# ShuhangGu/DASR

Hardware: NVIDIA B200
Metric: x4 SR output megapixels/sec (RRDBNet-23 G forward) (higher is better)
Workload: dtype bf16

## Files before the change

### dasr_b200/csrc/conv_tc.cu

```cuda
#include <stdlib.h>
#include "tc_common.cuh"

namespace dasr {

constexpr int EPI_WGS = 2;
constexpr int EPI_WARPS = 4 * EPI_WGS;
constexpr int MMA_WARPS = 1;
constexpr int TCK_WARPS = 2 + EPI_WARPS + 1 + (MMA_WARPS - 1);
constexpr int TCK_THREADS = 32 * TCK_WARPS;

struct EpiMaps {
  CUtensorMap m[8];
};

struct TcKernelArgs {
  DasrConvTcParams p;
  const float* bias;
  const __nv_bfloat16* res1;
  const __nv_bfloat16* res2;
  const __nv_bfloat16* mask_src;
  void* out;
  int nchunks;
  int chunk64;
  int nloads;
  int n_ntiles;
  int tiles_x, tiles_y;
  long ntiles;
  int stages;
  int w_bytes;
  int a_stage_bytes;
  int tmem_cols;
  int nacc;
  int acc_stride;
  int epi_bytes;
  int has_pre, has_res1, has_res2;
  int nbuf;
};


template <int EPI_MODE, bool HAS_PRE, int NRES>
__global__ void __launch_bounds__(TCK_THREADS, 1)
conv_tc_kernel(const __grid_constant__ CUtensorMap tmap_in, const __grid_constant__ CUtensorMap tmap_w,
               const __grid_constant__ EpiMaps em, const TcKernelArgs a) {
  extern __shared__ __align__(1024) uint8_t smem_raw[];
  uint8_t* smem = reinterpret_cast<uint8_t*>((reinterpret_cast<uintptr_t>(smem_raw) + 1023) & ~uintptr_t(1023));
  uint8_t* sW = smem;
  uint8_t* sA = smem + a.w_bytes;
  const int nbuf = a.nbuf;
  uint8_t* sS = sA + (size_t)a.stages * a.a_stage_bytes;
  uint8_t* sR1 = sS + nbuf * a.epi_bytes;
  uint8_t* sR2 = sR1 + (NRES >= 1 ? nbuf * a.epi_bytes : 0);
  uint64_t* bars = reinterpret_cast<uint64_t*>(sR2 + (NRES >= 2 ? nbuf * a.epi_bytes : 0));
  uint64_t* full_bar = bars;
  uint64_t* empty_bar = bars + MAX_STAGES;
  uint64_t* w_bar = bars + 2 * MAX_STAGES;
  uint64_t* tfull_bar = bars + 2 * MAX_STAGES + 1;
  uint64_t* tempty_bar = bars + 2 * MAX_STAGES + 5;
  uint64_t* pre_bar = bars + 2 * MAX_STAGES + 9;
  uint64_t* sfull_bar = bars + 2 * MAX_STAGES + 13;
  uint64_t* sfree_bar = bars + 2 * MAX_STAGES + 17;
  uint32_t* tmem_ptr = reinterpret_cast<uint32_t*>(bars + 2 * MAX_STAGES + 21);
  float* sBias = reinterpret_cast<float*>(bars + 2 * MAX_STAGES + 22);

  const DasrConvTcParams& p = a.p;
  const int warp = threadIdx.x >> 5, lane = threadIdx.x & 31;
  const int var = blockIdx.y / a.n_ntiles;
  const int ntile = blockIdx.y - var * a.n_ntiles;
  const int nt = p.nt;
  const int ntaps = p.ntaps;
  const int acc_stride = a.acc_stride;
  const uint32_t nacc = (uint32_t)a.nacc;
  const int nb64 = nt >> 6;
  const bool tail32 = (nt & 32) != 0;
  const bool has_loads = (EPI_MODE == 0) && (HAS_PRE || NRES > 0);

  if (threadIdx.x == 0) {
    tma_prefetch_desc(&tmap_in);
    tma_prefetch_desc(&tmap_w);
    for (int s = 0; s < a.stages; s++) {
      mbar_init(&full_bar[s], 1);
      mbar_init(&empty_bar[s], 1);
    }
    mbar_init(w_bar, 1);
    for (int b = 0; b < 4; b++) {
      mbar_init(&tfull_bar[b], 1);
      mbar_init(&tempty_bar[b], EPI_WARPS);
    }
    for (int b = 0; b < 4; b++) {
      mbar_init(&pre_bar[b], 1);
      mbar_init(&sfull_bar[b], EPI_WARPS);
      mbar_init(&sfree_bar[b], 1);
    }
    fence_barrier_init();
  }
  if (warp == 1) tmem_alloc(tmem_ptr, (uint32_t)a.tmem_cols);
  for (int i = threadIdx.x; i < nt; i += TCK_THREADS) sBias[i] = a.bias ? a.bias[ntile * nt + i] : 0.f;
  tc_fence_before();
  __syncthreads();
  tc_fence_after();
  const uint32_t tmem_base = *tmem_ptr;
  pdl_launch_dependents();

  if (warp == 0) {
    if (lane == 0) {
      mbar_expect_tx(w_bar, (uint32_t)a.w_bytes);
      for (int tap = 0; tap < ntaps; tap++)
        for (int c = 0; c < a.nchunks; c++) {
          int slot = tap * a.nchunks + c;
          int row = ((var * ntaps + tap) * a.nchunks + c) * p.cout + ntile * nt;
          tma_load_2d(sW + (size_t)slot * nt * ROW_B, &tmap_w, w_bar, 0, row);
        }
    }
    int stage = 0;
    uint32_t phase = 0;
    if (lane == 0) pdl_wait();
    __syncwarp();
    for (long tile = blockIdx.x; tile < a.ntiles; tile += gridDim.x) {
      const uint32_t te = (uint32_t)(p.tile_rev ? a.ntiles - 1 - tile : tile);
      const uint32_t r = te / (uint32_t)a.tiles_x;
      const int tx = (int)(te - r * (uint32_t)a.tiles_x);
      const int n = (int)(r / (uint32_t)a.tiles_y);
      const int ty = (int)(r - (uint32_t)n * (uint32_t)a.tiles_y);
      int x0 = tx * TILE_W, y0 = ty * TILE_H;
      if (lane == 0) {
        for (int c = 0; c < a.nloads; c++) {
          mbar_wait(&empty_bar[stage], phase ^ 1);
          uint8_t* dst = sA + (size_t)stage * a.a_stage_bytes;
          if (a.chunk64) {
            mbar_expect_tx(&full_bar[stage], 2 * A_HALO_BYTES);
            tma_load_4d(dst, &tmap_in, &full_bar[stage], p.in_coff + c * 2 * CHUNK, x0 - 1, y0 - 1, n);
          } else if (p.a_mode == 0) {
            mbar_expect_tx(&full_bar[stage], A_HALO_BYTES);
            tma_load_4d(dst, &tmap_in, &full_bar[stage], p.nchunk_list ? p.chunk_off[c] : p.in_coff + c * CHUNK, x0 - 1, y0 - 1, n);
          } else {
            mbar_expect_tx(&full_bar[stage], (uint32_t)(ntaps * A_TAP_BYTES));
            for (int tap = 0; tap < ntaps; tap++)
              tma_load_4d(dst + (size_t)tap * A_TAP_BYTES, &tmap_in, &full_bar[stage], p.nchunk_list ? p.chunk_off[c] : p.in_coff + c * CHUNK,
                          x0 - 1 + p.tap_dx[var][tap], y0 - 1 + p.tap_dy[var][tap], n);
          }
          if (++stage == a.stages) { stage = 0; phase ^= 1; }
        }
      }
      __syncwarp();
    }
  } else if (warp == 1 || (MMA_WARPS > 1 && warp == TCK_WARPS - 1)) {
    const uint32_t mi = (warp == 1) ? 0u : 1u;
    const uint32_t idesc = make_idesc_16(128, nt, p.f16);
    const uint32_t a_row = a.chunk64 ? 2u * ROW_B : (uint32_t)ROW_B;
    const uint32_t a_sbo = (p.a_mode == 0 && EPI_MODE != 3) ? (uint32_t)HALO_W * a_row : 8u * a_row;
    const uint64_t a_hi = ((uint64_t)((a_sbo >> 4) & 0x3FFF) << 32) | ((uint64_t)1 << 46) | ((uint64_t)(a.chunk64 ? 2 : 4) << 61) | ((uint64_t)1 << 16);
    const int ksteps = a.chunk64 ? 4 : 2;
    const uint64_t b_hi = ((uint64_t)(((8 * ROW_B) >> 4) & 0x3FFF) << 32) | ((uint64_t)1 << 46) | ((uint64_t)4 << 61) | ((uint64_t)1 << 16);
    const uint32_t a_lo0 = smem_u32(sA) >> 4;
    const uint32_t a_stage_lo = (uint32_t)a.a_stage_bytes >> 4;
    const uint32_t b_lo0 = smem_u32(sW) >> 4;
    const uint32_t b_slot_lo = (uint32_t)(nt * ROW_B) >> 4;
    uint32_t tap_lo[9];
#pragma unroll
    for (int t = 0; t < 9; t++) {
      int tt = t < ntaps ? t : 0;
      tap_lo[t] = (p.a_mode == 0) ? ((uint32_t)(p.tap_dy[var][tt] * HALO_W + p.tap_dx[var][tt]) * a_row) >> 4
                                  : (uint32_t)(tt * A_TAP_BYTES) >> 4;
    }
    mbar_wait(w_bar, 0);
    tc_fence_after();
    int stage = 0;
    uint32_t phase = 0;
    uint32_t it = 0;
    for (long tile = blockIdx.x; tile < a.ntiles; tile += gridDim.x, it++) {
      if ((it % MMA_WARPS) != mi) {
        for (int c = 0; c < a.nloads; c++)
          if (++stage == a.stages) { stage = 0; phase ^= 1; }
        continue;
      }
      const int acc = (int)(it % nacc);
      const uint32_t acc_phase = (it / nacc) & 1;
      mbar_wait(&tempty_bar[acc], acc_phase ^ 1);
      tc_fence_after();
      const uint32_t d_tmem = tmem_base + (uint32_t)(acc * acc_stride);
      for (int c = 0; c < a.nloads; c++) {
        mbar_wait(&full_bar[stage], phase);
        tc_fence_after();
        if (elect_one()) {
          const uint32_t a_lo = a_lo0 + (uint32_t)stage * a_stage_lo;
          const uint32_t b_tap_step = (uint32_t)a.nchunks * b_slot_lo;
          const uint32_t cb = a.chunk64 ? 2u * (uint32_t)c : (uint32_t)c;
          if constexpr (EPI_MODE == 3) {
#pragma unroll
            for (int mh = 0; mh < 2; mh++) {
              const uint32_t al = a_lo + (uint32_t)mh * ((128u * a_row) >> 4);
              for (int ks = 0; ks < ksteps; ks++) {
                const uint32_t bl = b_lo0 + (cb + (uint32_t)(ks >> 1)) * b_slot_lo + 2u * (uint32_t)(ks & 1);
                umma_bf16(d_tmem + (uint32_t)mh * 32u, a_hi | (uint64_t)((al + 2u * ks) & 0x3FFF), b_hi | (uint64_t)(bl & 0x3FFF), idesc,
                          (uint32_t)((c | ks) != 0));
              }
            }
          } else {
#pragma unroll
            for (int tap = 0; tap < 9; tap++) {
              if (tap < ntaps) {
                const uint32_t al = a_lo + tap_lo[tap];
                for (int ks = 0; ks < ksteps; ks++) {
                  const uint32_t bl = b_lo0 + (cb + (uint32_t)(ks >> 1)) * b_slot_lo + (uint32_t)tap * b_tap_step + 2u * (uint32_t)(ks & 1);
                  umma_bf16(d_tmem, a_hi | (uint64_t)((al + 2u * ks) & 0x3FFF), b_hi | (uint64_t)(bl & 0x3FFF), idesc,
                            (uint32_t)((c | tap | ks) != 0));
                }
              }
            }
          }
          umma_commit(&empty_bar[stage]);
          if (c == a.nloads - 1) umma_commit(&tfull_bar[acc]);
        }
        __syncwarp();
        if (++stage == a.stages) { stage = 0; phase ^= 1; }
      }
    }
  } else if (warp == TCK_WARPS - MMA_WARPS) {
    if constexpr (EPI_MODE == 0) {
      const int co_base = p.out_coff + ntile * nt;
      const int omap = (p.out_mul == 2) ? 2 * var : 0;
      const uint32_t load_bytes = (uint32_t)(((HAS_PRE ? 1 : 0) + NRES) * a.epi_bytes);
      pdl_wait();
      auto tile_xyz = [&](long tile, int& x0, int& y0, int& n) {
        const uint32_t te = (uint32_t)(p.tile_rev ? a.ntiles - 1 - tile : tile);
        const uint32_t r = te / (uint32_t)a.tiles_x;
        const int tx = (int)(te - r * (uint32_t)a.tiles_x);
        n = (int)(r / (uint32_t)a.tiles_y);
        const int ty = (int)(r - (uint32_t)n * (uint32_t)a.tiles_y);
        x0 = tx * TILE_W;
        y0 = ty * TILE_H;
      };
      auto issue_loads = [&](long tile, int b) {
        int x0, y0, n;
        tile_xyz(tile, x0, y0, n);
        if (lane == 0) {
          mbar_expect_tx(&pre_bar[b], load_bytes);
          const int cb = ntile * nt;
          for (int i = 0; i < nb64 + (tail32 ? 1 : 0); i++) {
            const int wide = i < nb64;
            const int off = wide ? i * EPI_BLK64_BYTES : nb64 * EPI_BLK64_BYTES;
            const int col = cb + (wide ? i * 64 : nb64 * 64);
            if constexpr (HAS_PRE) tma_load_4d(sS + b * a.epi_bytes + off, &em.m[wide ? 2 : 3], &pre_bar[b], p.pre_coff + col, x0, y0, n);
            if constexpr (NRES >= 1) tma_load_4d(sR1 + b * a.epi_bytes + off, &em.m[wide ? 4 : 5], &pre_bar[b], p.res1_coff + col, x0, y0, n);
            if constexpr (NRES >= 2) tma_load_4d(sR2 + b * a.epi_bytes + off, &em.m[wide ? 6 : 7], &pre_bar[b], p.res2_coff + col, x0, y0, n);
          }
        }
        __syncwarp();
      };
      const long G = gridDim.x;
      if (has_loads) {
        for (int k = 0; k < nbuf; k++)
          if ((long)blockIdx.x + k * G < a.ntiles) issue_loads(blockIdx.x + k * G, k);
      }
      uint32_t it = 0;
      long prev_tile = -1;
      int prev_b = 0;
      auto retire = [&](long t, int bb) {
        if (has_loads) {
          if (t + (long)nbuf * G < a.ntiles) issue_loads(t + (long)nbuf * G, bb);
        } else if (lane == 0) {
          mbar_arrive(&sfree_bar[bb]);
        }
        __syncwarp();
      };
      for (long tile = blockIdx.x; tile < a.ntiles; tile += G, it++) {
        const int b = (int)(it % (uint32_t)nbuf);
        if (lane == 0) {
          int x0, y0, n;
          tile_xyz(tile, x0, y0, n);
          mbar_wait(&sfull_bar[b], (it / (uint32_t)nbuf) & 1);
          for (int i = 0; i < nb64 + (tail32 ? 1 : 0); i++) {
            const int wide = i < nb64;
            const int off = wide ? i * EPI_BLK64_BYTES : nb64 * EPI_BLK64_BYTES;
            tma_store_4d(&em.m[(wide ? 0 : 1) + omap], sS + b * a.epi_bytes + off, co_base + (wide ? i * 64 : nb64 * 64), x0, y0, n);
          }
          bulk_commit();
          if (prev_tile >= 0) asm volatile("cp.async.bulk.wait_group.read 1;" ::: "memory");
        }
        __syncwarp();
        if (prev_tile >= 0) retire(prev_tile, prev_b);
        prev_tile = tile;
        prev_b = b;
      }
      if (prev_tile >= 0) {
        if (lane == 0) bulk_wait_read0();
        __syncwarp();
        retire(prev_tile, prev_b);
      }
      if (lane == 0) bulk_wait0();
    }
  } else {
    if constexpr (EPI_MODE != 0) pdl_wait();
    const int ew = warp - 2;
    const int wg = ew >> 2;
    const int q = warp & 3;
    const int m = q * 32 + lane;
    const int py = m >> 3, px = m & 7;
    const int co_base = ntile * nt;
    const int OW = p.W * p.out_mul, OH = p.H * p.out_mul;
    const int ngroups = nt >> 4;
    const int act = p.act, f16 = p.f16;
    const float slope = p.slope, alpha = p.alpha;
    const bool scale = alpha != 1.f;
    const int sw64 = (m >> 1) & 3, sw128 = m & 7;
    const uint32_t sS_u = smem_u32(sS), sR1_u = smem_u32(sR1), sR2_u = smem_u32(sR2), sBias_u = smem_u32(sBias);
    const bool has_bias = a.bias != nullptr;
    uint32_t it = 0;
    const int g0 = wg, gs = EPI_WGS;
    for (long tile = blockIdx.x; tile < a.ntiles; tile += gridDim.x, it++) {
      const int acc = (int)(it % nacc);
      const uint32_t acc_phase = (it / nacc) & 1;
      const uint32_t te = (uint32_t)(p.tile_rev ? a.ntiles - 1 - tile : tile);
      const uint32_t r = te / (uint32_t)a.tiles_x;
      const int tx = (int)(te - r * (uint32_t)a.tiles_x);
      const int n = (int)(r / (uint32_t)a.tiles_y);
      const int ty = (int)(r - (uint32_t)n * (uint32_t)a.tiles_y);
      const int y = ty * TILE_H + py, x = tx * TILE_W + px;
      const bool valid = (y < p.H) && (x < p.W);
      const int oy = y * p.out_mul + p.out_py[var], ox = x * p.out_mul + p.out_px[var];
      const long opix = ((long)n * OH + oy) * OW + ox;
      const int sb = (int)(it % (uint32_t)nbuf);
      const uint32_t sphase = (it / (uint32_t)nbuf) & 1;
      const uint32_t bS = sS_u + sb * a.epi_bytes, bR1 = sR1_u + sb * a.epi_bytes, bR2 = sR2_u + sb * a.epi_bytes;

      mbar_wait(&tfull_bar[acc], acc_phase);
      tc_fence_after();
      if constexpr (EPI_MODE == 0) {
        if (has_loads) mbar_wait(&pre_bar[sb], sphase);
        else if (it >= (uint32_t)nbuf) mbar_wait(&sfree_bar[sb], sphase ^ 1);
      }
      const uint32_t t_addr = tmem_base + ((uint32_t)(q * 32) << 16) + (uint32_t)(acc * acc_stride);
      if constexpr (EPI_MODE == 3) {
        float* S = reinterpret_cast<float*>(sS);
        constexpr int SROW = 29;
        const int hrow = wg * 128 + m;
        uint32_t r0[16], r1[16];
        tmem_ld16(t_addr + wg * 32, r0);
        tmem_ld16(t_addr + wg * 32 + 16, r1);
        tmem_ld_wait();
        tc_fence_before();
        __syncwarp();
        if (lane == 0) mbar_arrive(&tempty_bar[acc]);
        if (hrow < HALO_W * HALO_H) {
#pragma unroll
          for (int j = 0; j < 16; j++) S[hrow * SROW + j] = __uint_as_float(r0[j]);
#pragma unroll
          for (int j = 0; j < 11; j++) S[hrow * SROW + 16 + j] = __uint_as_float(r1[j]);
        }
        asm volatile("bar.sync 1, %0;" ::"n"(EPI_WARPS * 32) : "memory");
        if (wg == 0 && valid) {
          float* of = reinterpret_cast<float*>(a.out);
          const long plane = (long)OH * OW;
          const int onc = p.out_nc;
          for (int c = 0; c < onc; c++) {
            float v = has_bias ? sBias[c] : 0.f;
#pragma unroll
            for (int t9 = 0; t9 < 9; t9++) v += S[((py + t9 / 3) * HALO_W + (px + t9 % 3)) * SROW + t9 * onc + c];
            if (act != DASR_ACT_NONE && p.act_cols > 0) v = (act == DASR_ACT_LRELU) ? fmaxf(v, v * slope) : fmaxf(v, 0.f);
            of[((long)n * onc + c) * plane + (long)oy * OW + ox] = v * alpha;
          }
        }
        asm volatile("bar.sync 1, %0;" ::"n"(EPI_WARPS * 32) : "memory");
        continue;
      }
      auto process = [&](const uint32_t* rr, int g) {
        const int cg = g << 4;
        const int co = co_base + cg;
        const bool do_act = (act != DASR_ACT_NONE) && (co + 16 <= p.act_cols);
        float v[16];
#pragma unroll
        for (int j = 0; j < 16; j++) v[j] = __uint_as_float(rr[j]);
        if (has_bias) {
#pragma unroll
          for (int j4 = 0; j4 < 4; j4++) {
            const float4 b4 = lds128f(sBias_u + (cg + 4 * j4) * 4);
            v[4 * j4 + 0] += b4.x;
            v[4 * j4 + 1] += b4.y;
            v[4 * j4 + 2] += b4.z;
            v[4 * j4 + 3] += b4.w;
          }
        }
        if constexpr (EPI_MODE == 0) {
          int o0, o1;
          if (cg < (nb64 << 6)) {
            const int base = (cg >> 6) * EPI_BLK64_BYTES + m * 128;
            const int c0 = (cg & 63) >> 3;
            o0 = base + ((c0 ^ sw128) << 4);
            o1 = base + (((c0 + 1) ^ sw128) << 4);
          } else {
            const int base = nb64 * EPI_BLK64_BYTES + m * 64;
            const int c0 = (cg & 31) >> 3;
            o0 = base + ((c0 ^ sw64) << 4);
            o1 = base + (((c0 + 1) ^ sw64) << 4);
          }
          if constexpr (HAS_PRE) {
            fma_h16x8(v, lds128(bS + o0), 1.f, f16);
            fma_h16x8(v + 8, lds128(bS + o1), 1.f, f16);
          }
          if (do_act) {
            if (act == DASR_ACT_LRELU) {
#pragma unroll
              for (int j = 0; j < 16; j++) v[j] = fmaxf(v[j], v[j] * slope);
            } else {
#pragma unroll
              for (int j = 0; j < 16; j++) v[j] = fmaxf(v[j], 0.f);
            }
          }
          if (scale) {
#pragma unroll
            for (int j = 0; j < 16; j++) v[j] *= alpha;
          }
          if constexpr (NRES >= 1) {
            fma_h16x8(v, lds128(bR1 + o0), p.beta1, f16);
            fma_h16x8(v + 8, lds128(bR1 + o1), p.beta1, f16);
          }
          if constexpr (NRES >= 2) {
            fma_h16x8(v, lds128(bR2 + o0), p.beta2, f16);
            fma_h16x8(v + 8, lds128(bR2 + o1), p.beta2, f16);
          }
          uint4 o[2];
          pack_h16x16(v, o, f16);
          sts128(bS + o0, o[0]);
          sts128(bS + o1, o[1]);
        } else if (valid) {
          if (do_act) {
#pragma unroll
            for (int j = 0; j < 16; j++) v[j] = (act == DASR_ACT_LRELU) ? fmaxf(v[j], v[j] * slope) : fmaxf(v[j], 0.f);
          }
#pragma unroll
          for (int j = 0; j < 16; j++) v[j] *= alpha;
          if constexpr (EPI_MODE == 2) {
            float* of = reinterpret_cast<float*>(a.out);
            const long plane = (long)OH * OW;
#pragma unroll
            for (int j = 0; j < 16; j++)
              if (co + j < p.out_nc) of[((long)n * p.out_nc + co + j) * plane + (long)oy * OW + ox] = v[j];
          } else {
            __nv_bfloat16* ob16 = reinterpret_cast<__nv_bfloat16*>(a.out);
            if (a.res1) {
              const uint4* rp = reinterpret_cast<const uint4*>(a.res1 + opix * p.res1_cs + p.res1_coff + co);
              fma_h16x8(v, __ldg(rp), p.beta1, f16);
              fma_h16x8(v + 8, __ldg(rp + 1), p.beta1, f16);
            }
            if (a.res2) {
              const uint4* rp = reinterpret_cast<const uint4*>(a.res2 + opix * p.res2_cs + p.res2_coff + co);
              fma_h16x8(v, __ldg(rp), p.beta2, f16);
              fma_h16x8(v + 8, __ldg(rp + 1), p.beta2, f16);
            }
            if (a.mask_src && co + 16 > p.mask_c0 && co < p.mask_c1) {
              const __nv_bfloat16* mp = a.mask_src + opix * p.mask_cs + p.mask_coff + (co - p.mask_c0);
#pragma unroll
              for (int j = 0; j < 16; j++) {
                int cc = co + j;
                if (cc >= p.mask_c0 && cc < p.mask_c1) {
                  float mv = __bfloat162float(mp[j]);
                  if (!(mv > 0.f)) v[j] *= p.mask_slope;
                }
              }
            }
            uint4 o[2];
            pack_h16x16(v, o, f16);
            uint4* op = reinterpret_cast<uint4*>(ob16 + opix * p.out_cs + p.out_coff + co);
            op[0] = o[0];
            op[1] = o[1];
          }
        }
      };
      auto release_acc = [&]() {
        tc_fence_before();
        __syncwarp();
        if (lane == 0) mbar_arrive(&tempty_bar[acc]);
      };
      uint32_t ra[16], rb[16];
      if (g0 < ngroups) tmem_ld16(t_addr + g0 * 16, ra);
      for (int g = g0; g < ngroups; g += 2 * gs) {
        tmem_ld_wait();
        if (g + gs < ngroups) tmem_ld16(t_addr + (g + gs) * 16, rb); else release_acc();
        process(ra, g);
        if (g + gs < ngroups) {
          tmem_ld_wait();
          if (g + 2 * gs < ngroups) tmem_ld16(t_addr + (g + 2 * gs) * 16, ra); else release_acc();
          process(rb, g + gs);
        }
      }
      if (g0 >= ngroups) {
        tc_fence_before();
        __syncwarp();
        if (lane == 0) mbar_arrive(&tempty_bar[acc]);
      }
      if constexpr (EPI_MODE == 0) {
        fence_proxy_async();
        __syncwarp();
        if (lane == 0) mbar_arrive(&sfull_bar[sb]);
      }
    }
  }

  tc_fence_before();
  __syncthreads();
  if (warp == 1) {
    tc_fence_after();
    tmem_dealloc(tmem_base, (uint32_t)a.tmem_cols);
  }
}

__global__ void pack_filter_tc_kernel(const float* __restrict__ w, unsigned short* __restrict__ o, int cout, int cin,
                                      int kind, int f16) {
  const int gn = (kind == 1) ? cin : cout;
  const int gk = (kind == 1) ? cout : cin;
  if (kind == 3) {
    const long total3 = (long)(cin / CHUNK) * 32 * CHUNK;
    const long i3 = (long)blockIdx.x * blockDim.x + threadIdx.x;
    if (i3 >= total3) return;
    const int kc3 = (int)(i3 % CHUNK), n3 = (int)((i3 / CHUNK) % 32), c3 = (int)(i3 / (CHUNK * 32));
    float v3 = 0.f;
    if (n3 < 9 * cout) {
      const int tap = n3 / cout, co = n3 - tap * cout;
      v3 = w[((long)co * cin + c3 * CHUNK + kc3) * 9 + tap];
    }
    o[i3] = f16 ? __half_as_ushort(__float2half_rn(v3)) : __bfloat16_as_ushort(__float2bfloat16(v3));
    return;
  }
  const int nvar = (kind == 2) ? 4 : 1, ntaps = (kind == 2) ? 4 : 9, nchunks = gk / CHUNK;
  long total = (long)nvar * ntaps * nchunks * gn * CHUNK;
  long i = (long)blockIdx.x * blockDim.x + threadIdx.x;
  if (i >= total) return;
  int kc = (int)(i % CHUNK);
  long r = i / CHUNK;
  int nn = (int)(r % gn); r /= gn;
  int c = (int)(r % nchunks); r /= nchunks;
  int tap = (int)(r % ntaps);
  int var = (int)(r / ntaps);
  int kk = c * CHUNK + kc;
  float v = 0.f;
  if (kind == 0) {
    v = w[((long)nn * cin + kk) * 9 + tap];
  } else if (kind == 1) {
    int dy = tap / 3, dx = tap % 3;
    v = w[((long)kk * cin + nn) * 9 + (2 - dy) * 3 + (2 - dx)];
  } else {
    int py = var >> 1, px = var & 1, ta = tap >> 1, tb = tap & 1;
    int r0, r1, c0, c1;
    if (py == 0) { r0 = ta ? 1 : 0; r1 = ta ? 2 : 0; } else { r0 = ta ? 2 : 0; r1 = ta ? 2 : 1; }
    if (px == 0) { c0 = tb ? 1 : 0; c1 = tb ? 2 : 0; } else { c0 = tb ? 2 : 0; c1 = tb ? 2 : 1; }
    for (int rr = r0; rr <= r1; rr++)
      for (int cc = c0; cc <= c1; cc++) v += w[((long)nn * cin + kk) * 9 + rr * 3 + cc];
  }
  o[i] = f16 ? __half_as_ushort(__float2half_rn(v)) : __bfloat16_as_ushort(__float2bfloat16(v));
}

__global__ void pack_filter_tc_batch_kernel(const DasrPackJob* __restrict__ jobs) {
  const DasrPackJob j = jobs[blockIdx.y];
  if (j.kind == 3) {
    float* d = reinterpret_cast<float*>(j.dst);
    for (long i = (long)blockIdx.x * blockDim.x + threadIdx.x; i < j.cout; i += (long)gridDim.x * blockDim.x) d[i] = j.src[i];
    return;
  }
  const int rows = (j.kind == 1) ? j.ci_n : j.cout_rows;
  const int gk = (j.kind == 1) ? j.k_pad : j.ci_n;
  const int nvar = (j.kind == 2) ? 4 : 1, ntaps = (j.kind == 2) ? 4 : 9, nchunks = gk / CHUNK;
  const long total = (long)nvar * ntaps * nchunks * rows * CHUNK;
  __nv_bfloat16* o = reinterpret_cast<__nv_bfloat16*>(j.dst);
  for (long i = (long)blockIdx.x * blockDim.x + threadIdx.x; i < total; i += (long)gridDim.x * blockDim.x) {
    int kc = (int)(i % CHUNK);
    long r = i / CHUNK;
    int nn = (int)(r % rows); r /= rows;
    int c = (int)(r % nchunks); r /= nchunks;
    int tap = (int)(r % ntaps);
    int var = (int)(r / ntaps);
    int kk = c * CHUNK + kc;
    float v = 0.f;
    if (j.kind == 0) {
      if (nn < j.cout && j.ci_lo + kk < j.cin) v = j.src[((long)nn * j.cin + j.ci_lo + kk) * 9 + tap];
    } else if (j.kind == 1) {
      int dy = tap / 3, dx = tap % 3;
      if (kk < j.cout && j.ci_lo + nn < j.cin) v = j.src[((long)kk * j.cin + j.ci_lo + nn) * 9 + (2 - dy) * 3 + (2 - dx)];
    } else {
      int py = var >> 1, px = var & 1, ta = tap >> 1, tb = tap & 1;
      int r0, r1, c0, c1;
      if (py == 0) { r0 = ta ? 1 : 0; r1 = ta ? 2 : 0; } else { r0 = ta ? 2 : 0; r1 = ta ? 2 : 1; }
      if (px == 0) { c0 = tb ? 1 : 0; c1 = tb ? 2 : 0; } else { c0 = tb ? 2 : 0; c1 = tb ? 2 : 1; }
      if (nn < j.cout && j.ci_lo + kk < j.cin)
        for (int rr = r0; rr <= r1; rr++)
          for (int cc = c0; cc <= c1; cc++) v += j.src[((long)nn * j.cin + j.ci_lo + kk) * 9 + rr * 3 + cc];
    }
    o[(((long)var * ntaps + tap) * nchunks + c) * j.dst_rows * CHUNK + (long)(j.dst_row_off + nn) * CHUNK + kc] = __float2bfloat16(v);
  }
}


static int pow2_at_least(int v) {
  int r = 32;
  while (r < v) r <<= 1;
  return r;
}


__global__ void __launch_bounds__(128, 1) mma_rate_kernel(int n, int sbo, int iters, int a_step, long long* out) {
  const int nacc = (a_step >> 16) & 15 ? (a_step >> 16) & 15 : 1;
  const bool nowait = (a_step >> 20) & 1;
  a_step &= 0xFFFF;
  extern __shared__ __align__(1024) uint8_t smem_raw[];
  uint8_t* smem = reinterpret_cast<uint8_t*>((reinterpret_cast<uintptr_t>(smem_raw) + 1023) & ~uintptr_t(1023));
  __shared__ uint64_t bar;
  __shared__ uint32_t tptr;
  for (int i = threadIdx.x; i < 48 * 1024 / 4; i += blockDim.x) reinterpret_cast<uint32_t*>(smem)[i] = 0;
  if (threadIdx.x == 0) { mbar_init(&bar, 1); fence_barrier_init(); }
  fence_proxy_async();
  if (threadIdx.x < 32) tmem_alloc(&tptr, 512);
  tc_fence_before();
  __syncthreads();
  tc_fence_after();
  const uint32_t tb = tptr;
  if (threadIdx.x < 32) {
    const uint32_t idesc = make_idesc_bf16(128, n);
    const uint32_t a0 = smem_u32(smem), b0 = smem_u32(smem + 16384);
    const uint32_t acc_stride = 512u / (uint32_t)nacc;
    long long t0 = clock64();
    uint32_t ph = 0;
    for (int it = 0; it < iters; it++) {
      if (elect_one()) {
        int kk = 0;
#pragma unroll 1
        for (int tap = 0; tap < 9; tap++) {
          uint32_t aa = a0 + (uint32_t)(((tap / 3) * 10 + (tap % 3)) * a_step);
#pragma unroll
          for (int k = 0; k < 2; k++, kk++)
            umma_bf16(tb + (uint32_t)(kk % nacc) * acc_stride, make_desc_sw64(aa + k * 32, (uint32_t)sbo),
                      make_desc_sw64(b0 + k * 32, 512), idesc, 1u);
        }
        if (!nowait || it == iters - 1) umma_commit(&bar);
      }
      __syncwarp();
      if (!nowait || it == iters - 1) {
        mbar_wait(&bar, ph);
        ph ^= 1;
      }
    }
    long long t1 = clock64();
    if (threadIdx.x == 0 && blockIdx.x == 0) out[0] = (t1 - t0);
  }
  tc_fence_before();
  __syncthreads();
  if (threadIdx.x < 32) { tc_fence_after(); tmem_dealloc(tb, 512); }
}

__global__ void __launch_bounds__(64, 1) tma_rate_kernel(const __grid_constant__ CUtensorMap tm, int rows_per_box,
                                                         int box_bytes, int iters, int store, long npix, long long* out) {
  extern __shared__ __align__(1024) uint8_t smem_raw[];
  uint8_t* smem = reinterpret_cast<uint8_t*>((reinterpret_cast<uintptr_t>(smem_raw) + 1023) & ~uintptr_t(1023));
  __shared__ uint64_t bar[4];
  if (threadIdx.x == 0) {
    for (int i = 0; i < 4; i++) mbar_init(&bar[i], 1);
    fence_barrier_init();
  }
  __syncthreads();
  if (threadIdx.x == 0) {
    const int nbox = (int)(npix / rows_per_box);
    long long t0 = clock64();
    if (!store) {
      uint32_t ph[4] = {0, 0, 0, 0};
      for (int i = 0; i < iters + 4; i++) {
        int s = i & 3;
        if (i >= 4) { mbar_wait(&bar[s], ph[s]); ph[s] ^= 1; }
        if (i < iters) {
          int b = (int)(((long)blockIdx.x * 7919 + (long)i * 104729) % nbox);
          mbar_expect_tx(&bar[s], (uint32_t)box_bytes);
          tma_load_2d(smem + s * 49152, &tm, &bar[s], 0, b * rows_per_box);
        }
      }
    } else {
      for (int i = 0; i < iters; i++) {
        int b = (int)(((long)blockIdx.x * 7919 + (long)i * 104729) % nbox);
        asm volatile("cp.async.bulk.tensor.2d.global.shared::cta.bulk_group [%0, {%2, %3}], [%1];" ::"l"(
                         reinterpret_cast<uint64_t>(&tm)), "r"(smem_u32(smem + (i & 3) * 49152)), "r"(0), "r"(b * rows_per_box)
                     : "memory");
        bulk_commit();
        asm volatile("cp.async.bulk.wait_group.read 3;" ::: "memory");
      }
      bulk_wait0();
    }
    long long t1 = clock64();
    if (blockIdx.x == 0) out[0] = t1 - t0;
  }
}

}

using namespace dasr;

extern "C" {

int dasr_conv_tc_setup(DasrConvTcParams* p, int kind) {
  if (!p) return DASR_E_BADARG;
  p->nchunk_list = 0;
  p->f16 = 0;
  if (kind == 0 || kind == 1) {
    p->nvar = 1;
    p->ntaps = 9;
    p->out_mul = 1;
    for (int t = 0; t < 9; t++) {
      p->tap_dy[0][t] = (int8_t)(t / 3);
      p->tap_dx[0][t] = (int8_t)(t % 3);
    }
    p->out_py[0] = p->out_px[0] = 0;
  } else if (kind == 2) {
    p->nvar = 4;
    p->ntaps = 4;
    p->out_mul = 2;
    for (int v = 0; v < 4; v++) {
      int py = v >> 1, px = v & 1;
      p->out_py[v] = py;
      p->out_px[v] = px;
      for (int t = 0; t < 4; t++) {
        p->tap_dy[v][t] = (int8_t)(py + (t >> 1));
        p->tap_dx[v][t] = (int8_t)(px + (t & 1));
      }
    }
  } else if (kind == 3) {
    p->nvar = 1;
    p->ntaps = 1;
    p->out_mul = 1;
    p->tap_dy[0][0] = p->tap_dx[0][0] = 0;
    p->out_py[0] = p->out_px[0] = 0;
  } else {
    set_error("conv_tc_setup: unknown kind %d", kind);
    return DASR_E_BADARG;
  }
  return DASR_OK;
}

size_t dasr_pack_filter_tc_bytes(int cout, int cin, int kind) {
  if (kind == 3) return (size_t)(cin / CHUNK) * 32 * CHUNK * 2;
  int nvar = (kind == 2) ? 4 : 1, ntaps = (kind == 2) ? 4 : 9;
  return (size_t)nvar * ntaps * cout * cin * 2;
}

int dasr_pack_filter_tc(const float* w, void* o, int cout, int cin, int kind, void* stream) {
  const int f16 = (kind & DASR_TC_PACK_F16) != 0;
  kind &= ~DASR_TC_PACK_F16;
  DASR_REQUIRE(kind >= 0 && kind <= 3, "pack_filter_tc: kind");
  DASR_REQUIRE(kind != 3 || (cout >= 1 && 9 * cout <= 32), "pack_filter_tc: kind 3 (taps in N) needs cout <= 3");
  int gk = (kind == 1) ? cout : cin;
  DASR_REQUIRE(gk % CHUNK == 0, "pack_filter_tc: contraction channels (%d) must be a multiple of 32", gk);
  long total = (long)dasr_pack_filter_tc_bytes(cout, cin, kind) / 2;
  pack_filter_tc_kernel<<<cdiv(total, 256), 256, 0, (cudaStream_t)stream>>>(w, (unsigned short*)o, cout, cin, kind, f16);
  return check_launch("pack_filter_tc");
}

int dasr_pack_filter_tc_batch(const DasrPackJob* jobs_dev, int njobs, int blocks_per_job, void* stream) {
  DASR_REQUIRE(jobs_dev && njobs > 0 && njobs <= 65535 && blocks_per_job > 0, "pack_filter_tc_batch: bad arguments");
  dim3 grid(blocks_per_job, njobs);
  pack_filter_tc_batch_kernel<<<grid, 256, 0, (cudaStream_t)stream>>>(jobs_dev);
  return check_launch("pack_filter_tc_batch");
}

static int encode_act_map(PFN_encodeTiled enc, CUtensorMap* tm, const void* base, int cs, int W, int H, int N,
                          int width, const char* what, int mul = 1) {
  cuuint64_t gdim[4] = {(cuuint64_t)cs, (cuuint64_t)W, (cuuint64_t)H, (cuuint64_t)N};
  cuuint64_t gstr[3] = {(cuuint64_t)mul * cs * 2, (cuuint64_t)mul * (mul * W) * cs * 2, (cuuint64_t)(mul * H) * (mul * W) * cs * 2};
  cuuint32_t box[4] = {(cuuint32_t)width, TILE_W, TILE_H, 1};
  cuuint32_t estr[4] = {1, 1, 1, 1};
  CUresult r = enc(tm, CU_TENSOR_MAP_DATA_TYPE_BFLOAT16, 4, const_cast<void*>(base), gdim, gstr, box, estr,
                   CU_TENSOR_MAP_INTERLEAVE_NONE, width == 64 ? CU_TENSOR_MAP_SWIZZLE_128B : CU_TENSOR_MAP_SWIZZLE_64B,
                   (width == 32 && cs > 32) ? CU_TENSOR_MAP_L2_PROMOTION_L2_64B : CU_TENSOR_MAP_L2_PROMOTION_L2_128B,
                   CU_TENSOR_MAP_FLOAT_OOB_FILL_NONE);
  if (r != CUDA_SUCCESS) {
    set_error("conv_tc: cuTensorMapEncodeTiled(%s) failed: %d", what, (int)r);
    return DASR_E_LAUNCH;
  }
  return DASR_OK;
}

int dasr_conv_tc(const void* in, const void* w, const float* bias, const void* pre, const void* res1, const void* res2,
                 const void* mask_src, void* out, const DasrConvTcParams* p, void* stream) {
  DASR_REQUIRE(p && in && w && out, "conv_tc: null argument");
  DASR_REQUIRE(p->N > 0 && p->H > 0 && p->W > 0, "conv_tc: bad dims");
  DASR_REQUIRE((long)p->N * cdiv(p->W, TILE_W) * cdiv(p->H, TILE_H) < (1L << 30), "conv_tc: too many tiles for 32-bit tile arithmetic");
  DASR_REQUIRE(p->cin > 0 && p->cin % CHUNK == 0, "conv_tc: cin must be a multiple of 32 (got %d)", p->cin);
  if (p->nchunk_list > 0) {
    DASR_REQUIRE(p->nchunk_list <= 8 && p->nchunk_list * CHUNK == p->cin && p->in_cs % 8 == 0, "conv_tc: chunk list must cover cin");
    for (int i = 0; i < p->nchunk_list; i++)
      DASR_REQUIRE(p->chunk_off[i] >= 0 && p->chunk_off[i] % 8 == 0 && p->chunk_off[i] + CHUNK <= p->in_cs, "conv_tc: chunk_off[%d]", i);
  } else {
    DASR_REQUIRE(p->in_cs % 8 == 0 && p->in_coff % 8 == 0 && p->in_coff + p->cin <= p->in_cs, "conv_tc: input slice");
  }
  DASR_REQUIRE(p->nt >= 16 && p->nt <= 256 && p->nt % 16 == 0 && p->cout % p->nt == 0, "conv_tc: nt=%d cout=%d",
               p->nt, p->cout);
  DASR_REQUIRE(p->nvar >= 1 && p->nvar <= 4 && p->ntaps >= 1 && p->ntaps <= 9, "conv_tc: variants/taps");
  DASR_REQUIRE(p->out_mul == 1 || p->out_mul == 2, "conv_tc: out_mul");
  DASR_REQUIRE(p->epi_mode >= 0 && p->epi_mode <= 3, "conv_tc: epi_mode");
  DASR_REQUIRE(p->f16 == 0 || (p->f16 == 1 && !mask_src), "conv_tc: f16 must be 0/1; the dgrad mask input is bf16 only");
  DASR_REQUIRE(p->act_cols % 16 == 0, "conv_tc: act_cols must be a multiple of 16");
  if (p->epi_mode == 2) {
    DASR_REQUIRE(p->out_nc >= 1 && p->out_nc <= 16 && p->nt == p->cout && !res1 && !res2 && !pre && !mask_src,
                 "conv_tc: NCHW-fp32 epilogue supports out_nc<=16, one Cout tile, no residuals");
  } else if (p->epi_mode == 3) {
    DASR_REQUIRE(p->out_nc >= 1 && 9 * p->out_nc <= 32 && p->nt == 32 && p->cout == 32 && p->ntaps == 1 && p->nvar == 1 &&
                     p->a_mode == 0 && p->out_mul == 1 && !res1 && !res2 && !pre && !mask_src && !p->tile_rev,
                 "conv_tc: epi_mode 3 (taps in N, NCHW fp32 out) needs dasr_conv_tc_setup kind 3, out_nc <= 3, nt = cout = 32");
  } else {
    DASR_REQUIRE(p->out_cs % 8 == 0 && p->out_coff % 8 == 0 && p->out_coff + p->cout <= p->out_cs, "conv_tc: output slice");
  }
  if (p->epi_mode == 0) {
    DASR_REQUIRE(p->nt % 32 == 0 && !mask_src, "conv_tc: staged epilogue needs nt%%32==0, no mask");
    DASR_REQUIRE(p->out_mul == 1 || (!pre && !res1 && !res2),
                 "conv_tc: the staged epilogue of the sub-pixel (out_mul=2) variants has no pre / residual inputs");
  } else {
    DASR_REQUIRE(!pre, "conv_tc: the pre-activation addend is only supported by the staged epilogue (epi_mode 0)");
  }
  if (res1) DASR_REQUIRE(p->res1_cs % 8 == 0 && p->res1_coff % 8 == 0, "conv_tc: res1 alignment");
  if (res2) DASR_REQUIRE(p->res2_cs % 8 == 0 && p->res2_coff % 8 == 0, "conv_tc: res2 alignment");
  if (pre) DASR_REQUIRE(p->pre_cs % 8 == 0 && p->pre_coff % 8 == 0, "conv_tc: pre alignment");
  DASR_REQUIRE((reinterpret_cast<uintptr_t>(in) & 15) == 0 && (reinterpret_cast<uintptr_t>(out) & 15) == 0 &&
                   (reinterpret_cast<uintptr_t>(w) & 15) == 0,
               "conv_tc: pointers must be 16-byte aligned");
  PFN_encodeTiled enc = get_encode();
  if (!enc) {
    set_error("conv_tc: cuTensorMapEncodeTiled not available");
    return DASR_E_NODRIVER;
  }

  TcKernelArgs a;
  a.p = *p;
  a.bias = bias;
  a.res1 = (const __nv_bfloat16*)res1;
  a.res2 = (const __nv_bfloat16*)res2;
  a.mask_src = (const __nv_bfloat16*)mask_src;
  a.out = out;
  a.nchunks = p->cin / CHUNK;
  a.n_ntiles = p->cout / p->nt;
  a.tiles_x = cdiv(p->W, TILE_W);
  a.tiles_y = cdiv(p->H, TILE_H);
  a.ntiles = (long)p->N * a.tiles_x * a.tiles_y;
  a.w_bytes = p->ntaps * a.nchunks * p->nt * ROW_B;
  static int chunk64_ok = -1;
  if (chunk64_ok < 0) {
    const char* e = getenv("DASR_TC_CHUNK64");
    chunk64_ok = (e && e[0] == '0') ? 0 : 1;
  }
  a.chunk64 = (chunk64_ok && p->a_mode == 0 && p->nchunk_list == 0 && p->cin % (2 * CHUNK) == 0) ? 1 : 0;
  a.nloads = a.chunk64 ? a.nchunks / 2 : a.nchunks;
  a.a_stage_bytes = (p->a_mode == 0) ? (((a.chunk64 ? 2 : 1) * A_HALO_BYTES + 1023) / 1024 * 1024) : p->ntaps * A_TAP_BYTES;
  a.acc_stride = (p->epi_mode == 3) ? 64 : pow2_at_least(p->nt);
  a.nacc = (a.acc_stride <= 128) ? 4 : 2;
  a.tmem_cols = a.nacc * a.acc_stride;
  if (a.tmem_cols < 32) a.tmem_cols = 32;
  a.has_pre = (p->epi_mode == 0 && pre) ? 1 : 0;
  a.has_res1 = (p->epi_mode == 0 && res1) ? 1 : 0;
  a.has_res2 = (p->epi_mode == 0 && res2) ? 1 : 0;
  a.epi_bytes = (p->epi_mode == 0) ? p->nt * 128 * 2 : (p->epi_mode == 3 ? 21504 : 0);
  const int bar_bytes = (2 * MAX_STAGES + 22) * 8 + 256 * 4 + 16;
  int nbuf = (p->epi_mode == 0) ? 4 : (p->epi_mode == 3 ? 1 : 2);
  int epi_total = 0, avail = 0;
  for (;; nbuf--) {
    epi_total = nbuf * a.epi_bytes * (1 + a.has_res1 + a.has_res2);
    avail = SMEM_LIMIT - 1024  - a.w_bytes - epi_total - bar_bytes;
    if (nbuf <= 2 || avail >= 4 * a.a_stage_bytes) break;
  }
  a.nbuf = nbuf;
  int stages = avail / a.a_stage_bytes;
  if (stages > MAX_STAGES) stages = MAX_STAGES;
  if (stages < 2) {
    set_error("conv_tc: resident filters (%d B) + epilogue tiles (%d B) + 2 A stages do not fit shared memory; use a smaller nt",
              a.w_bytes, epi_total);
    return DASR_E_SMEM;
  }
  a.stages = stages;
  size_t smem = 1024 + (size_t)a.w_bytes + (size_t)stages * a.a_stage_bytes + epi_total + bar_bytes;
  if (smem < 120 * 1024) smem = 120 * 1024;

  CUtensorMap tm_in, tm_w;
  EpiMaps em;
  {
    cuuint64_t gdim[4] = {(cuuint64_t)p->in_cs, (cuuint64_t)p->W, (cuuint64_t)p->H, (cuuint64_t)p->N};
    cuuint64_t gstr[3] = {(cuuint64_t)p->in_cs * 2, (cuuint64_t)p->W * p->in_cs * 2,
                          (cuuint64_t)p->H * p->W * p->in_cs * 2};
    cuuint32_t box[4] = {(cuuint32_t)(a.chunk64 ? 2 * CHUNK : CHUNK), (cuuint32_t)(p->a_mode == 0 ? HALO_W : TILE_W),
                         (cuuint32_t)(p->a_mode == 0 ? HALO_H : TILE_H), 1};
    cuuint32_t estr[4] = {1, 1, 1, 1};
    CUresult r = enc(&tm_in, CU_TENSOR_MAP_DATA_TYPE_BFLOAT16, 4, const_cast<void*>(in), gdim, gstr, box, estr,
                     CU_TENSOR_MAP_INTERLEAVE_NONE, a.chunk64 ? CU_TENSOR_MAP_SWIZZLE_128B : CU_TENSOR_MAP_SWIZZLE_64B,
                     (p->in_cs > CHUNK && !a.chunk64) ? CU_TENSOR_MAP_L2_PROMOTION_L2_64B : CU_TENSOR_MAP_L2_PROMOTION_L2_128B,
                     CU_TENSOR_MAP_FLOAT_OOB_FILL_NONE);
    if (r != CUDA_SUCCESS) {
      set_error("conv_tc: cuTensorMapEncodeTiled(input) failed: %d", (int)r);
      return DASR_E_LAUNCH;
    }
  }
  {
    cuuint64_t rows = (cuuint64_t)p->nvar * p->ntaps * a.nchunks * p->cout;
    cuuint64_t gdim[2] = {CHUNK, rows};
    cuuint64_t gstr[1] = {ROW_B};
    cuuint32_t box[2] = {CHUNK, (cuuint32_t)p->nt};
    cuuint32_t estr[2] = {1, 1};
    CUresult r = enc(&tm_w, CU_TENSOR_MAP_DATA_TYPE_BFLOAT16, 2, const_cast<void*>(w), gdim, gstr, box, estr,
                     CU_TENSOR_MAP_INTERLEAVE_NONE, CU_TENSOR_MAP_SWIZZLE_64B, CU_TENSOR_MAP_L2_PROMOTION_L2_128B,
                     CU_TENSOR_MAP_FLOAT_OOB_FILL_NONE);
    if (r != CUDA_SUCCESS) {
      set_error("conv_tc: cuTensorMapEncodeTiled(filter) failed: %d", (int)r);
      return DASR_E_LAUNCH;
    }
  }
  for (int i = 0; i < 8; i++) em.m[i] = tm_in;
  if (p->epi_mode == 0) {
    const void* bases[4] = {out, pre, res1, res2};
    const int css[4] = {p->out_cs, p->pre_cs, p->res1_cs, p->res2_cs};
    const int used[4] = {1, a.has_pre, a.has_res1, a.has_res2};
    const char* names[4] = {"output", "pre", "res1", "res2"};
    if (p->out_mul == 2) {
      for (int v = 0; v < p->nvar && v < 4; v++) {
        const char* vb = (const char*)out + ((size_t)p->out_py[v] * (2 * p->W) + p->out_px[v]) * p->out_cs * 2;
        int rc;
        if (p->nt >= 64 && (rc = encode_act_map(enc, &em.m[2 * v], vb, p->out_cs, p->W, p->H, p->N, 64, "output", 2))) return rc;
        if ((p->nt & 32) && (rc = encode_act_map(enc, &em.m[2 * v + 1], vb, p->out_cs, p->W, p->H, p->N, 32, "output", 2))) return rc;
      }
    } else
    for (int t = 0; t < 4; t++) {
      if (!used[t]) continue;
      int rc;
      if (p->nt >= 64 && (rc = encode_act_map(enc, &em.m[2 * t], bases[t], css[t], p->W, p->H, p->N, 64, names[t]))) return rc;
      if ((p->nt & 32) && (rc = encode_act_map(enc, &em.m[2 * t + 1], bases[t], css[t], p->W, p->H, p->N, 32, names[t]))) return rc;
    }
  }

  typedef void (*KernelFn)(const CUtensorMap, const CUtensorMap, const EpiMaps, const TcKernelArgs);
  static const KernelFn kernels[9] = {
      conv_tc_kernel<0, false, 0>, conv_tc_kernel<0, false, 1>, conv_tc_kernel<0, false, 2>,
      conv_tc_kernel<0, true, 0>,  conv_tc_kernel<0, true, 1>,  conv_tc_kernel<0, true, 2>,
      conv_tc_kernel<1, false, 0>, conv_tc_kernel<2, false, 0>, conv_tc_kernel<3, false, 0>};
  const int ki = (p->epi_mode == 0) ? (a.has_pre * 3 + a.has_res1 + a.has_res2) : (5 + p->epi_mode);
  if (p->epi_mode == 0) DASR_REQUIRE(!(a.has_res2 && !a.has_res1), "conv_tc: res2 without res1");
  static bool attr_set[9] = {false, false, false, false, false, false, false, false, false};
  if (!attr_set[ki]) {
    cudaError_t e = cudaFuncSetAttribute(kernels[ki], cudaFuncAttributeMaxDynamicSharedMemorySize, SMEM_LIMIT);
    if (e != cudaSuccess) {
      set_error("conv_tc: cudaFuncSetAttribute: %s", cudaGetErrorString(e));
      return DASR_E_LAUNCH;
    }
    attr_set[ki] = true;
  }
  int gy = p->nvar * a.n_ntiles;
  int gx = num_sms() / gy;
  if (gx < 1) gx = 1;
  if ((long)gx > a.ntiles) gx = (int)a.ntiles;
  cudaLaunchConfig_t cfg = {};
  cfg.gridDim = dim3(gx, gy, 1);
  cfg.blockDim = dim3(TCK_THREADS, 1, 1);
  cfg.dynamicSmemBytes = smem;
  cfg.stream = (cudaStream_t)stream;
  cudaLaunchAttribute attrs[1];
  attrs[0].id = cudaLaunchAttributeProgrammaticStreamSerialization;
  attrs[0].val.programmaticStreamSerializationAllowed = pdl_enabled() ? 1 : 0;
  cfg.attrs = attrs;
  cfg.numAttrs = 1;
  cudaError_t le = cudaLaunchKernelEx(&cfg, kernels[ki], tm_in, tm_w, em, a);
  if (le != cudaSuccess) {
    set_error("conv_tc: launch failed: %s", cudaGetErrorString(le));
    return DASR_E_LAUNCH;
  }
  return check_launch("conv_tc");
}

int dasr_probe_mma_rate(int n, int sbo, int iters, int a_step, double* cycles_per_mma) {
  long long* d;
  if (cudaMalloc(&d, 8) != cudaSuccess) return DASR_E_LAUNCH;
  cudaFuncSetAttribute(mma_rate_kernel, cudaFuncAttributeMaxDynamicSharedMemorySize, 64 * 1024);
  mma_rate_kernel<<<num_sms(), 128, 64 * 1024>>>(n, sbo, iters, a_step, d);
  long long h = 0;
  cudaError_t e = cudaMemcpy(&h, d, 8, cudaMemcpyDeviceToHost);
  cudaFree(d);
  if (e != cudaSuccess) { set_error("probe: %s", cudaGetErrorString(e)); return DASR_E_LAUNCH; }
  *cycles_per_mma = (double)h / ((double)iters * 18.0);
  return DASR_OK;
}


int dasr_probe_tma_rate(int row_elems, int rows_per_box, int cs, int store, double* cycles_per_box) {
  PFN_encodeTiled enc = get_encode();
  if (!enc) return DASR_E_NODRIVER;
  const long npix = 1L << 20;
  void* buf;
  if (cudaMalloc(&buf, (size_t)npix * cs * 2) != cudaSuccess) return DASR_E_LAUNCH;
  cudaMemset(buf, 0, (size_t)npix * cs * 2);
  CUtensorMap tm;
  cuuint64_t gdim[2] = {(cuuint64_t)cs, (cuuint64_t)npix};
  cuuint64_t gstr[1] = {(cuuint64_t)cs * 2};
  cuuint32_t box[2] = {(cuuint32_t)row_elems, (cuuint32_t)rows_per_box};
  cuuint32_t estr[2] = {1, 1};
  CUtensorMapSwizzle sw = row_elems * 2 == 64 ? CU_TENSOR_MAP_SWIZZLE_64B : (row_elems * 2 == 128 ? CU_TENSOR_MAP_SWIZZLE_128B : CU_TENSOR_MAP_SWIZZLE_NONE);
  CUresult r = enc(&tm, CU_TENSOR_MAP_DATA_TYPE_BFLOAT16, 2, buf, gdim, gstr, box, estr, CU_TENSOR_MAP_INTERLEAVE_NONE, sw,
                   CU_TENSOR_MAP_L2_PROMOTION_L2_128B, CU_TENSOR_MAP_FLOAT_OOB_FILL_NONE);
  if (r != CUDA_SUCCESS) { cudaFree(buf); set_error("probe tma: encode %d", (int)r); return DASR_E_LAUNCH; }
  long long* d;
  cudaMalloc(&d, 8);
  const int iters = 400;
  cudaFuncSetAttribute(tma_rate_kernel, cudaFuncAttributeMaxDynamicSharedMemorySize, 200 * 1024);
  tma_rate_kernel<<<num_sms(), 64, 200 * 1024>>>(tm, rows_per_box, row_elems * 2 * rows_per_box, iters, store, npix, d);
  long long h = 0;
  cudaError_t e = cudaMemcpy(&h, d, 8, cudaMemcpyDeviceToHost);
  cudaFree(d);
  cudaFree(buf);
  if (e != cudaSuccess) { set_error("probe tma: %s", cudaGetErrorString(e)); return DASR_E_LAUNCH; }
  *cycles_per_box = (double)h / iters;
  return DASR_OK;
}

}
```

### dasr_b200/csrc/conv_tc2.cu

```cuda
#include <stdlib.h>
#include "tc_common.cuh"

namespace dasr {

constexpr int TC2_EPI_WARPS = 8;
constexpr int TC2_WARPS = 2 + TC2_EPI_WARPS + 1;
constexpr int TC2_THREADS = 32 * TC2_WARPS;
constexpr int TC2_MAX_STAGES = 6;
constexpr int TC2_MAX_BLOCKS = 6;

struct Tc2Maps {
  CUtensorMap m[8];
};

struct Tc2Args {
  DasrConvTcParams p;
  const float* bias;
  int nchunks;
  int n_half;
  int tiles_x, tiles_y;
  long ntiles;
  int stages, a_stage_bytes, w_bytes;
  int nblk;
  int nb64;
  int nb;
  int acc_stride;
};

template <bool HAS_PRE, int NRES>
__global__ void __cluster_dims__(2, 1, 1) __launch_bounds__(TC2_THREADS, 1)
conv_tc2_kernel(const __grid_constant__ CUtensorMap tmap_in, const __grid_constant__ CUtensorMap tmap_w,
                const __grid_constant__ Tc2Maps em, const Tc2Args a) {
  extern __shared__ __align__(1024) uint8_t smem_raw[];
  uint8_t* smem = reinterpret_cast<uint8_t*>((reinterpret_cast<uintptr_t>(smem_raw) + 1023) & ~uintptr_t(1023));
  uint8_t* sW = smem;
  uint8_t* sA = smem + a.w_bytes;
  uint8_t* sS = sA + (size_t)a.stages * a.a_stage_bytes;
  uint8_t* sR1 = sS + (size_t)a.nblk * EPI_BLK64_BYTES;
  uint8_t* sR2 = sR1 + (NRES >= 1 ? (size_t)a.nblk * EPI_BLK64_BYTES : 0);
  uint64_t* bars = reinterpret_cast<uint64_t*>(sR2 + (NRES >= 2 ? (size_t)a.nblk * EPI_BLK64_BYTES : 0));
  constexpr bool HAS_LOADS = HAS_PRE || NRES > 0;
  uint64_t* full_bar = bars;
  uint64_t* empty_bar = bars + TC2_MAX_STAGES;
  uint64_t* w_bar = bars + 2 * TC2_MAX_STAGES;
  uint64_t* tfull_bar = w_bar + 1;
  uint64_t* tempty_bar = tfull_bar + 2;
  uint64_t* sfull_bar = tempty_bar + 2;
  uint64_t* sfree_bar = sfull_bar + TC2_MAX_BLOCKS;
  uint64_t* pre_bar = sfree_bar + TC2_MAX_BLOCKS;
  uint32_t* tmem_ptr = reinterpret_cast<uint32_t*>(pre_bar + TC2_MAX_BLOCKS);
  float* sBias = reinterpret_cast<float*>(bars + 40);

  const DasrConvTcParams& p = a.p;
  const int warp = threadIdx.x >> 5, lane = threadIdx.x & 31;
  const uint32_t rank = cluster_ctarank();
  const long pair = blockIdx.x >> 1, npairs = gridDim.x >> 1;
  const int cout = p.nt;
  const int co_base = (int)blockIdx.y * p.nt;

  if (threadIdx.x == 0) {
    tma_prefetch_desc(&tmap_in);
    tma_prefetch_desc(&tmap_w);
    tma_prefetch_desc(&em.m[0]);
    for (int s = 0; s < a.stages; s++) {
      mbar_init(&full_bar[s], 1);
      mbar_init(&empty_bar[s], 1);
    }
    mbar_init(w_bar, 1);
    for (int b = 0; b < 2; b++) {
      mbar_init(&tfull_bar[b], 1);
      mbar_init(&tempty_bar[b], 2 * TC2_EPI_WARPS);
    }
    for (int b = 0; b < a.nblk; b++) {
      mbar_init(&sfull_bar[b], TC2_EPI_WARPS);
      mbar_init(&sfree_bar[b], 1);
      mbar_init(&pre_bar[b], 1);
    }
    fence_barrier_init();
  }
  for (int i = threadIdx.x; i < cout; i += TC2_THREADS) sBias[i] = a.bias ? a.bias[co_base + i] : 0.f;
  cluster_sync();
  if (warp == 1) tmem_alloc2(tmem_ptr, 512);
  tc_fence_before();
  __syncthreads();
  tc_fence_after();
  const uint32_t tmem_base = *tmem_ptr;
  pdl_launch_dependents();

  auto tile_of = [&](long it, int& x0, int& y0, int& n) -> bool {
    uint32_t t = 2u * (uint32_t)(pair + it * npairs) + rank;
    const bool live = (long)t < a.ntiles;
    if (p.tile_rev && live) t = (uint32_t)(a.ntiles - 1) - t;
    const uint32_t r = t / (uint32_t)a.tiles_x;
    const uint32_t tx = t - r * (uint32_t)a.tiles_x;
    n = (int)(r / (uint32_t)a.tiles_y);
    const uint32_t ty = r - (uint32_t)n * (uint32_t)a.tiles_y;
    x0 = (int)tx * TILE_W;
    y0 = (int)ty * TILE_H;
    return live;
  };
  const long niter = (a.ntiles / 2 + (a.ntiles & 1) - pair + npairs - 1) / npairs;

  if (warp == 0) {
    if (lane == 0) {
      if (rank == 0) mbar_expect_tx(w_bar, 2u * (uint32_t)a.w_bytes);
      for (int tap = 0; tap < 9; tap++)
        for (int c = 0; c < a.nchunks; c++) {
          const int slot = tap * a.nchunks + c;
          const int row = slot * p.cout + co_base + (int)rank * a.n_half;
          tma2_load_2d(sW + (size_t)slot * a.n_half * ROW_B, &tmap_w, w_bar, 0, row);
        }
      pdl_wait();
      int stage = 0;
      uint32_t phase = 0;
      for (long it = 0; it < niter; it++) {
        int x0, y0, n;
        tile_of(it, x0, y0, n);
        for (int c = 0; c < a.nchunks; c++) {
          mbar_wait(&empty_bar[stage], phase ^ 1);
          if (rank == 0) mbar_expect_tx(&full_bar[stage], 2u * A_HALO_BYTES);
          tma2_load_4d(sA + (size_t)stage * a.a_stage_bytes, &tmap_in, &full_bar[stage],
                       p.nchunk_list ? p.chunk_off[c] : p.in_coff + c * CHUNK, x0 - 1, y0 - 1, n);
          if (++stage == a.stages) { stage = 0; phase ^= 1; }
        }
      }
    }
    __syncwarp();
  } else if (warp == 1) {
    if (rank == 0) {
      const uint32_t idesc = make_idesc_16(256, cout, p.f16);
      const uint32_t a_sbo = (uint32_t)(HALO_W * ROW_B);
      const uint64_t a_hi = ((uint64_t)((a_sbo >> 4) & 0x3FFF) << 32) | ((uint64_t)1 << 46) | ((uint64_t)4 << 61) | ((uint64_t)1 << 16);
      const uint64_t b_hi = ((uint64_t)(((8 * ROW_B) >> 4) & 0x3FFF) << 32) | ((uint64_t)1 << 46) | ((uint64_t)4 << 61) | ((uint64_t)1 << 16);
      const uint32_t a_lo0 = smem_u32(sA) >> 4;
      const uint32_t a_stage_lo = (uint32_t)a.a_stage_bytes >> 4;
      const uint32_t b_lo0 = smem_u32(sW) >> 4;
      const uint32_t b_slot_lo = (uint32_t)(a.n_half * ROW_B) >> 4;
      uint32_t tap_lo[9];
#pragma unroll
      for (int t = 0; t < 9; t++) tap_lo[t] = (uint32_t)(((t / 3) * HALO_W + (t % 3)) * ROW_B) >> 4;
      mbar_wait(w_bar, 0);
      tc_fence_after();
      int stage = 0;
      uint32_t phase = 0;
      for (long it = 0; it < niter; it++) {
        const int acc = (int)(it & 1);
        mbar_wait(&tempty_bar[acc], ((uint32_t)(it >> 1) & 1) ^ 1);
        tc_fence_after();
        const uint32_t d_tmem = tmem_base + (uint32_t)(acc * a.acc_stride);
        for (int c = 0; c < a.nchunks; c++) {
          mbar_wait(&full_bar[stage], phase);
          tc_fence_after();
          if (elect_one()) {
            const uint32_t a_lo = a_lo0 + (uint32_t)stage * a_stage_lo;
            uint32_t b_lo = b_lo0 + (uint32_t)c * b_slot_lo;
            const uint32_t b_tap_step = (uint32_t)a.nchunks * b_slot_lo;
#pragma unroll
            for (int tap = 0; tap < 9; tap++) {
              const uint32_t al = a_lo + tap_lo[tap];
              umma2_bf16(d_tmem, a_hi | (uint64_t)(al & 0x3FFF), b_hi | (uint64_t)(b_lo & 0x3FFF), idesc, (uint32_t)((c | tap) != 0));
              umma2_bf16(d_tmem, a_hi | (uint64_t)((al + 2) & 0x3FFF), b_hi | (uint64_t)((b_lo + 2) & 0x3FFF), idesc, 1u);
              b_lo += b_tap_step;
            }
            umma2_commit_mc(&empty_bar[stage]);
            if (c == a.nchunks - 1) umma2_commit_mc(&tfull_bar[acc]);
          }
          __syncwarp();
          if (++stage == a.stages) { stage = 0; phase ^= 1; }
        }
      }
    }
  } else if (warp == TC2_WARPS - 1) {
    if (lane == 0) {
      pdl_wait();
      const uint32_t nb = (uint32_t)a.nb, nblk = (uint32_t)a.nblk;
      const uint32_t total = (uint32_t)niter * nb;
      const uint32_t nld = (uint32_t)((HAS_PRE ? 1 : 0) + NRES);
      const bool mask_mode = (NRES >= 1) && (p.mask_c1 > p.mask_c0);
      auto issue_loads = [&](uint32_t k) {
        const uint32_t b = k % nblk;
        int x0, y0, n;
        const uint32_t kt = k / nb;
        tile_of((long)kt, x0, y0, n);
        const int i = (int)(k - kt * nb);
        const int wide = i < a.nb64 ? 1 : 0;
        const int col = co_base + i * 64;
        const bool need_r1 = !mask_mode || (col < p.mask_c1 && col + (wide ? 64 : 32) > p.mask_c0);
        mbar_expect_tx(&pre_bar[b], (nld - (need_r1 ? 0u : 1u)) * (uint32_t)(wide ? EPI_BLK64_BYTES : EPI_BLK32_BYTES));
        if constexpr (HAS_PRE) tma_load_4d(sS + (size_t)b * EPI_BLK64_BYTES, &em.m[wide ? 2 : 3], &pre_bar[b], p.pre_coff + col, x0, y0, n);
        if constexpr (NRES >= 1) {
          if (need_r1) tma_load_4d(sR1 + (size_t)b * EPI_BLK64_BYTES, &em.m[wide ? 4 : 5], &pre_bar[b], p.res1_coff + col, x0, y0, n);
        }
        if constexpr (NRES >= 2) tma_load_4d(sR2 + (size_t)b * EPI_BLK64_BYTES, &em.m[wide ? 6 : 7], &pre_bar[b], p.res2_coff + col, x0, y0, n);
      };
      if constexpr (HAS_LOADS)
        for (uint32_t k = 0; k < nblk && k < total; k++) issue_loads(k);
      auto retire = [&](uint32_t k) {
        if constexpr (HAS_LOADS) {
          if (k + nblk < total) issue_loads(k + nblk);
        } else {
          mbar_arrive(&sfree_bar[k % nblk]);
        }
      };
      int x0 = 0, y0 = 0, n = 0;
      bool live = false;
      uint32_t i = 0;
      for (uint32_t k = 0; k < total; k++) {
        const uint32_t b = k % nblk;
        if (i == 0) live = tile_of((long)(k / nb), x0, y0, n);
        mbar_wait(&sfull_bar[b], (k / nblk) & 1);
        if (live) tma_store_4d(&em.m[(int)i < a.nb64 ? 0 : 1], sS + (size_t)b * EPI_BLK64_BYTES, p.out_coff + co_base + (int)i * 64, x0, y0, n);
        bulk_commit();
        if (k >= 1) {
          asm volatile("cp.async.bulk.wait_group.read 1;" ::: "memory");
          retire(k - 1);
        }
        if (++i == nb) i = 0;
      }
      if (total > 0) {
        bulk_wait_read0();
        retire(total - 1);
      }
      bulk_wait0();
    }
    __syncwarp();
  } else {
    const int ew = warp - 2;
    const int wg = ew >> 2;
    const int q = warp & 3;
    const int m = q * 32 + lane;
    const int sw128 = m & 7, sw64 = (m >> 1) & 3;
    const int act = p.act, f16 = p.f16;
    const float slope = p.slope, alpha = p.alpha;
    const bool scale = alpha != 1.f;
    const uint32_t sS_u = smem_u32(sS), sR1_u = smem_u32(sR1), sR2_u = smem_u32(sR2), sBias_u = smem_u32(sBias);
    const bool has_bias = a.bias != nullptr;
    uint32_t k = 0;
    for (long it = 0; it < niter; it++) {
      const int acc = (int)(it & 1);
      mbar_wait(&tfull_bar[acc], (uint32_t)(it >> 1) & 1);
      tc_fence_after();
      const uint32_t t_addr = tmem_base + ((uint32_t)(q * 32) << 16) + (uint32_t)(acc * a.acc_stride);
      for (int i = 0; i < a.nb; i++, k++) {
        const int b = (int)(k % (uint32_t)a.nblk);
        if constexpr (HAS_LOADS) {
          mbar_wait(&pre_bar[b], (k / (uint32_t)a.nblk) & 1);
        } else {
          if (k >= (uint32_t)a.nblk) mbar_wait(&sfree_bar[b], ((k / (uint32_t)a.nblk) & 1) ^ 1);
        }
        const bool wide = i < a.nb64;
        const uint32_t rowoff = (uint32_t)m * (wide ? 128u : 64u);
        const uint32_t bS = sS_u + (uint32_t)b * EPI_BLK64_BYTES + rowoff;
        const uint32_t bR1 = sR1_u + (uint32_t)b * EPI_BLK64_BYTES + rowoff;
        const uint32_t bR2 = sR2_u + (uint32_t)b * EPI_BLK64_BYTES + rowoff;
        uint32_t ra[16], rb[16];
        const int c0 = i * 64 + wg * 16, c1 = c0 + 32;
        tmem_ld16(t_addr + c0, ra);
        if (wide) tmem_ld16(t_addr + c1, rb);
        tmem_ld_wait();
        if (i == a.nb - 1) {
          tc_fence_before();
          __syncwarp();
          if (lane == 0) mbar_arrive_leader(&tempty_bar[acc]);
        }
#pragma unroll
        for (int h = 0; h < 2; h++) {
          if (h == 1 && !wide) break;
          const uint32_t* rr = h ? rb : ra;
          const int cg = h ? c1 : c0;
          const bool do_act = (act != DASR_ACT_NONE) && (co_base + cg + 16 <= p.act_cols);
          float v[16];
#pragma unroll
          for (int j = 0; j < 16; j++) v[j] = __uint_as_float(rr[j]);
          if (has_bias) {
#pragma unroll
            for (int j4 = 0; j4 < 4; j4++) {
              const float4 b4 = lds128f(sBias_u + (cg + 4 * j4) * 4);
              v[4 * j4 + 0] += b4.x;
              v[4 * j4 + 1] += b4.y;
              v[4 * j4 + 2] += b4.z;
              v[4 * j4 + 3] += b4.w;
            }
          }
          const int ch = (cg & (wide ? 63 : 31)) >> 3;
          const int sw = wide ? sw128 : sw64;
          const uint32_t o0 = (uint32_t)(((ch) ^ sw) << 4), o1 = (uint32_t)(((ch + 1) ^ sw) << 4);
          if constexpr (HAS_PRE) {
            fma_h16x8(v, lds128(bS + o0), 1.f, f16);
            fma_h16x8(v + 8, lds128(bS + o1), 1.f, f16);
          }
          if (do_act) {
            if (act == DASR_ACT_LRELU) {
#pragma unroll
              for (int j = 0; j < 16; j++) v[j] = fmaxf(v[j], v[j] * slope);
            } else {
#pragma unroll
              for (int j = 0; j < 16; j++) v[j] = fmaxf(v[j], 0.f);
            }
          }
          if (scale) {
#pragma unroll
            for (int j = 0; j < 16; j++) v[j] *= alpha;
          }
          if constexpr (NRES >= 1) {
            if (p.mask_c1 > p.mask_c0) {
              const int co = co_base + cg;
              if (co >= p.mask_c0 && co < p.mask_c1) {
                const uint4 m0 = lds128(bR1 + o0), m1 = lds128(bR1 + o1);
                const short* ms0 = reinterpret_cast<const short*>(&m0);
                const short* ms1 = reinterpret_cast<const short*>(&m1);
#pragma unroll
                for (int j = 0; j < 8; j++) {
                  if (!(ms0[j] > 0)) v[j] *= p.mask_slope;
                  if (!(ms1[j] > 0)) v[8 + j] *= p.mask_slope;
                }
              }
            } else {
              fma_h16x8(v, lds128(bR1 + o0), p.beta1, f16);
              fma_h16x8(v + 8, lds128(bR1 + o1), p.beta1, f16);
            }
          }
          if constexpr (NRES >= 2) {
            fma_h16x8(v, lds128(bR2 + o0), p.beta2, f16);
            fma_h16x8(v + 8, lds128(bR2 + o1), p.beta2, f16);
          }
          uint4 o[2];
          pack_h16x16(v, o, f16);
          sts128(bS + o0, o[0]);
          sts128(bS + o1, o[1]);
        }
        fence_proxy_async();
        __syncwarp();
        if (lane == 0) mbar_arrive(&sfull_bar[b]);
      }
    }
  }

  tc_fence_before();
  cluster_sync();
  if (warp == 1) {
    tc_fence_after();
    tmem_dealloc2(tmem_base, 512);
  }
}

__global__ void __cluster_dims__(2, 1, 1) __launch_bounds__(128, 1) mma2_rate_kernel(int n, int iters, long long* out) {
  extern __shared__ __align__(1024) uint8_t smem_raw[];
  uint8_t* smem = reinterpret_cast<uint8_t*>((reinterpret_cast<uintptr_t>(smem_raw) + 1023) & ~uintptr_t(1023));
  __shared__ uint64_t bar;
  __shared__ uint32_t tptr;
  for (int i = threadIdx.x; i < 48 * 1024 / 4; i += blockDim.x) reinterpret_cast<uint32_t*>(smem)[i] = 0;
  if (threadIdx.x == 0) { mbar_init(&bar, 1); fence_barrier_init(); }
  fence_proxy_async();
  cluster_sync();
  if (threadIdx.x < 32) tmem_alloc2(&tptr, 512);
  tc_fence_before();
  __syncthreads();
  tc_fence_after();
  const uint32_t tb = tptr;
  const uint32_t rank = cluster_ctarank();
  if (threadIdx.x < 32 && rank == 0) {
    const uint32_t idesc = make_idesc_bf16(256, n);
    const uint32_t a0 = smem_u32(smem), b0 = smem_u32(smem + 16384);
    long long t0 = clock64();
    for (int it = 0; it < iters; it++) {
      if (elect_one()) {
#pragma unroll 1
        for (int tap = 0; tap < 9; tap++) {
          uint32_t aa = a0 + (uint32_t)(((tap / 3) * 10 + (tap % 3)) * 64);
#pragma unroll
          for (int k = 0; k < 2; k++)
            umma2_bf16(tb, make_desc_sw64(aa + k * 32, 640), make_desc_sw64(b0 + k * 32, 512), idesc, 1u);
        }
        if (it == iters - 1)
          asm volatile("tcgen05.commit.cta_group::2.mbarrier::arrive::one.shared::cluster.b64 [%0];" ::"r"(smem_u32(&bar)) : "memory");
      }
      __syncwarp();
    }
    mbar_wait(&bar, 0);
    long long t1 = clock64();
    if (threadIdx.x == 0 && blockIdx.x == 0) out[0] = (t1 - t0);
  }
  tc_fence_before();
  cluster_sync();
  if (threadIdx.x < 32) { tc_fence_after(); tmem_dealloc2(tb, 512); }
}

}

using namespace dasr;

extern "C" {

static int tc2_plan(const DasrConvTcParams* p, int has_pre, int nres, int* stages_out, int* nblk_out) {
  const int nchunks = p->cin / CHUNK;
  const long w_bytes = (long)9 * nchunks * (p->nt / 2) * ROW_B;
  const int a_stage = (A_HALO_BYTES + 1023) / 1024 * 1024;
  const int bar_bytes = 40 * 8 + 256 * 4 + 64;
  const int per_blk = (1 + nres) * EPI_BLK64_BYTES;
  (void)has_pre;
  static int force_nblk = -1;
  if (force_nblk < 0) {
    const char* e = getenv("DASR_TC2_NBLK");
    force_nblk = e ? atoi(e) : 0;
  }
  for (int want = 4; want >= 2; want--)
    for (int nblk = TC2_MAX_BLOCKS; nblk >= 2; nblk--) {
      if (force_nblk > 0 && nblk != force_nblk) continue;
      const long avail = (long)SMEM_LIMIT - 1024 - w_bytes - (long)nblk * per_blk - bar_bytes;
      int stages = (int)(avail / a_stage);
      if (stages > TC2_MAX_STAGES) stages = TC2_MAX_STAGES;
      if (stages >= want) {
        *stages_out = stages;
        *nblk_out = nblk;
        return 1;
      }
    }
  return 0;
}

int dasr_conv_tc2_supported(const DasrConvTcParams* p) {
  if (!p) return 0;
  if (p->nvar != 1 || p->ntaps != 9 || p->out_mul != 1 || p->epi_mode != 0 || p->a_mode != 0) return 0;
  if (p->nt % 32 != 0 || p->nt < 32 || p->nt > 256 || p->cout % p->nt != 0 || p->cin % CHUNK != 0 || p->cin <= 0) return 0;
  int st, nb;
  const int nres = (p->res1_cs > 0 ? 1 : 0) + (p->res2_cs > 0 ? 1 : 0);
  return tc2_plan(p, p->pre_cs > 0 ? 1 : 0, nres, &st, &nb);
}

int dasr_conv_tc2(const void* in, const void* w, const float* bias, const void* pre, const void* res1, const void* res2,
                  void* out, const DasrConvTcParams* p, void* stream) {
  DASR_REQUIRE(p && in && w && out, "conv_tc2: null argument");
  DASR_REQUIRE(p->nvar == 1 && p->ntaps == 9 && p->out_mul == 1 && p->epi_mode == 0 && p->a_mode == 0,
               "conv_tc2: plain 3x3 geometry with the staged epilogue only");
  DASR_REQUIRE(p->nt % 32 == 0 && p->nt >= 32 && p->nt <= 256 && p->cout % p->nt == 0,
               "conv_tc2: the Cout tile nt must be a multiple of 32 in [32, 256] that divides cout (nt=%d cout=%d)", p->nt, p->cout);
  DASR_REQUIRE(p->N > 0 && p->H > 0 && p->W > 0, "conv_tc2: bad dims");
  DASR_REQUIRE((long)p->N * cdiv(p->W, TILE_W) * cdiv(p->H, TILE_H) < (1L << 30), "conv_tc2: too many tiles for 32-bit tile arithmetic");
  DASR_REQUIRE(p->cin > 0 && p->cin % CHUNK == 0, "conv_tc2: cin must be a multiple of 32 (got %d)", p->cin);
  if (p->nchunk_list > 0) {
    DASR_REQUIRE(p->nchunk_list <= 8 && p->nchunk_list * CHUNK == p->cin, "conv_tc2: chunk list must cover cin");
    for (int i = 0; i < p->nchunk_list; i++)
      DASR_REQUIRE(p->chunk_off[i] >= 0 && p->chunk_off[i] % 8 == 0 && p->chunk_off[i] + CHUNK <= p->in_cs, "conv_tc2: chunk_off[%d]", i);
  } else {
    DASR_REQUIRE(p->in_cs % 8 == 0 && p->in_coff % 8 == 0 && p->in_coff + p->cin <= p->in_cs, "conv_tc2: input slice");
  }
  DASR_REQUIRE(p->out_cs % 8 == 0 && p->out_coff % 8 == 0 && p->out_coff + p->cout <= p->out_cs, "conv_tc2: output slice");
  DASR_REQUIRE(p->act_cols % 16 == 0, "conv_tc2: act_cols must be a multiple of 16");
  DASR_REQUIRE(!(res2 && !res1), "conv_tc2: res2 without res1");
  if (p->mask_c1 > p->mask_c0)
    DASR_REQUIRE(res1 && !res2 && p->mask_c0 % 16 == 0 && p->mask_c1 % 16 == 0 && p->mask_c1 <= p->cout,
                 "conv_tc2: mask mode takes the activation as res1 (no res2) and a range of whole 16-channel groups");
  if (pre) DASR_REQUIRE(p->pre_cs % 8 == 0 && p->pre_coff % 8 == 0 && p->pre_coff + p->cout <= p->pre_cs, "conv_tc2: pre slice");
  if (res1) DASR_REQUIRE(p->res1_cs % 8 == 0 && p->res1_coff % 8 == 0 && p->res1_coff + p->cout <= p->res1_cs, "conv_tc2: res1 slice");
  if (res2) DASR_REQUIRE(p->res2_cs % 8 == 0 && p->res2_coff % 8 == 0 && p->res2_coff + p->cout <= p->res2_cs, "conv_tc2: res2 slice");
  PFN_encodeTiled enc = get_encode();
  if (!enc) {
    set_error("conv_tc2: cuTensorMapEncodeTiled not available");
    return DASR_E_NODRIVER;
  }
  const int has_pre = pre ? 1 : 0, nres = (res1 ? 1 : 0) + (res2 ? 1 : 0);
  Tc2Args a;
  a.p = *p;
  a.bias = bias;
  a.nchunks = p->cin / CHUNK;
  a.n_half = p->nt / 2;
  a.tiles_x = cdiv(p->W, TILE_W);
  a.tiles_y = cdiv(p->H, TILE_H);
  a.ntiles = (long)p->N * a.tiles_x * a.tiles_y;
  a.w_bytes = 9 * a.nchunks * a.n_half * ROW_B;
  a.a_stage_bytes = (A_HALO_BYTES + 1023) / 1024 * 1024;
  a.nb64 = p->nt / 64;
  a.nb = a.nb64 + ((p->nt & 32) ? 1 : 0);
  a.acc_stride = 256;
  const int bar_bytes = 40 * 8 + 256 * 4 + 64;
  int stages = 0, nblk = 0;
  if (!tc2_plan(p, has_pre, nres, &stages, &nblk)) {
    set_error("conv_tc2: filters (%d B per CTA) + %d epilogue block arrays do not fit shared memory", a.w_bytes, 1 + nres);
    return DASR_E_SMEM;
  }
  a.stages = stages;
  a.nblk = nblk;
  size_t smem = 1024 + (size_t)a.w_bytes + (size_t)stages * a.a_stage_bytes + (size_t)nblk * (1 + nres) * EPI_BLK64_BYTES + bar_bytes;
  if (smem < 120 * 1024) smem = 120 * 1024;

  CUtensorMap tm_in, tm_w;
  Tc2Maps em;
  {
    cuuint64_t gdim[4] = {(cuuint64_t)p->in_cs, (cuuint64_t)p->W, (cuuint64_t)p->H, (cuuint64_t)p->N};
    cuuint64_t gstr[3] = {(cuuint64_t)p->in_cs * 2, (cuuint64_t)p->W * p->in_cs * 2, (cuuint64_t)p->H * p->W * p->in_cs * 2};
    cuuint32_t box[4] = {CHUNK, HALO_W, HALO_H, 1};
    cuuint32_t estr[4] = {1, 1, 1, 1};
    CUresult r = enc(&tm_in, CU_TENSOR_MAP_DATA_TYPE_BFLOAT16, 4, const_cast<void*>(in), gdim, gstr, box, estr,
                     CU_TENSOR_MAP_INTERLEAVE_NONE, CU_TENSOR_MAP_SWIZZLE_64B,
                     p->in_cs > CHUNK ? CU_TENSOR_MAP_L2_PROMOTION_L2_64B : CU_TENSOR_MAP_L2_PROMOTION_L2_128B,
                     CU_TENSOR_MAP_FLOAT_OOB_FILL_NONE);
    if (r != CUDA_SUCCESS) { set_error("conv_tc2: cuTensorMapEncodeTiled(input) failed: %d", (int)r); return DASR_E_LAUNCH; }
  }
  {
    cuuint64_t rows = (cuuint64_t)9 * a.nchunks * p->cout;
    cuuint64_t gdim[2] = {CHUNK, rows};
    cuuint64_t gstr[1] = {ROW_B};
    cuuint32_t box[2] = {CHUNK, (cuuint32_t)a.n_half};
    cuuint32_t estr[2] = {1, 1};
    CUresult r = enc(&tm_w, CU_TENSOR_MAP_DATA_TYPE_BFLOAT16, 2, const_cast<void*>(w), gdim, gstr, box, estr,
                     CU_TENSOR_MAP_INTERLEAVE_NONE, CU_TENSOR_MAP_SWIZZLE_64B, CU_TENSOR_MAP_L2_PROMOTION_L2_128B,
                     CU_TENSOR_MAP_FLOAT_OOB_FILL_NONE);
    if (r != CUDA_SUCCESS) { set_error("conv_tc2: cuTensorMapEncodeTiled(filter) failed: %d", (int)r); return DASR_E_LAUNCH; }
  }
  {
    const void* bases[4] = {out, pre, res1, res2};
    const int css[4] = {p->out_cs, p->pre_cs, p->res1_cs, p->res2_cs};
    const char* names[4] = {"output", "pre", "res1", "res2"};
    for (int t = 0; t < 4; t++) {
      em.m[2 * t] = em.m[2 * t + 1] = tm_in;
      if (!bases[t]) continue;
      for (int narrow = 0; narrow < 2; narrow++) {
        if (narrow ? !(p->nt & 32) : (a.nb64 == 0)) continue;
        const int width = narrow ? 32 : 64;
        cuuint64_t gdim[4] = {(cuuint64_t)css[t], (cuuint64_t)p->W, (cuuint64_t)p->H, (cuuint64_t)p->N};
        cuuint64_t gstr[3] = {(cuuint64_t)css[t] * 2, (cuuint64_t)p->W * css[t] * 2, (cuuint64_t)p->H * p->W * css[t] * 2};
        cuuint32_t box[4] = {(cuuint32_t)width, TILE_W, TILE_H, 1};
        cuuint32_t estr[4] = {1, 1, 1, 1};
        CUresult r = enc(&em.m[2 * t + narrow], CU_TENSOR_MAP_DATA_TYPE_BFLOAT16, 4, const_cast<void*>(bases[t]), gdim, gstr, box, estr,
                         CU_TENSOR_MAP_INTERLEAVE_NONE, narrow ? CU_TENSOR_MAP_SWIZZLE_64B : CU_TENSOR_MAP_SWIZZLE_128B,
                         (narrow && css[t] > 32) ? CU_TENSOR_MAP_L2_PROMOTION_L2_64B : CU_TENSOR_MAP_L2_PROMOTION_L2_128B,
                         CU_TENSOR_MAP_FLOAT_OOB_FILL_NONE);
        if (r != CUDA_SUCCESS) { set_error("conv_tc2: cuTensorMapEncodeTiled(%s) failed: %d", names[t], (int)r); return DASR_E_LAUNCH; }
      }
    }
  }
  typedef void (*KernelFn)(const CUtensorMap, const CUtensorMap, const Tc2Maps, const Tc2Args);
  static const KernelFn kernels[6] = {conv_tc2_kernel<false, 0>, conv_tc2_kernel<false, 1>, conv_tc2_kernel<false, 2>,
                                      conv_tc2_kernel<true, 0>,  conv_tc2_kernel<true, 1>,  conv_tc2_kernel<true, 2>};
  const int ki = has_pre * 3 + nres;
  static bool attr_set[6] = {false, false, false, false, false, false};
  if (!attr_set[ki]) {
    cudaError_t e = cudaFuncSetAttribute(kernels[ki], cudaFuncAttributeMaxDynamicSharedMemorySize, SMEM_LIMIT);
    if (e != cudaSuccess) { set_error("conv_tc2: cudaFuncSetAttribute: %s", cudaGetErrorString(e)); return DASR_E_LAUNCH; }
    attr_set[ki] = true;
  }
  long npairs = (a.ntiles + 1) / 2;
  int gx = num_sms() & ~1;
  if ((long)gx > 2 * npairs) gx = (int)(2 * npairs);
  cudaLaunchConfig_t cfg = {};
  cfg.gridDim = dim3(gx, p->cout / p->nt, 1);
  cfg.blockDim = dim3(TC2_THREADS, 1, 1);
  cfg.dynamicSmemBytes = smem;
  cfg.stream = (cudaStream_t)stream;
  cudaLaunchAttribute attrs[1];
  attrs[0].id = cudaLaunchAttributeProgrammaticStreamSerialization;
  attrs[0].val.programmaticStreamSerializationAllowed = pdl_enabled() ? 1 : 0;
  cfg.attrs = attrs;
  cfg.numAttrs = 1;
  cudaError_t e = cudaLaunchKernelEx(&cfg, kernels[ki], tm_in, tm_w, em, a);
  if (e != cudaSuccess) {
    set_error("conv_tc2: launch failed: %s", cudaGetErrorString(e));
    return DASR_E_LAUNCH;
  }
  return check_launch("conv_tc2");
}

int dasr_probe_mma2_rate(int n, int iters, double* cycles_per_mma) {
  long long* d;
  if (cudaMalloc(&d, 8) != cudaSuccess) return DASR_E_LAUNCH;
  cudaFuncSetAttribute(mma2_rate_kernel, cudaFuncAttributeMaxDynamicSharedMemorySize, 64 * 1024);
  mma2_rate_kernel<<<num_sms() & ~1, 128, 64 * 1024>>>(n, iters, d);
  long long h = 0;
  cudaError_t e = cudaMemcpy(&h, d, 8, cudaMemcpyDeviceToHost);
  cudaFree(d);
  if (e != cudaSuccess) { set_error("probe mma2: %s", cudaGetErrorString(e)); return DASR_E_LAUNCH; }
  *cycles_per_mma = (double)h / ((double)iters * 18.0);
  return DASR_OK;
}

}
```

### dasr_b200/csrc/selftest.cu

```cuda
#include <cuda_runtime.h>
#include <cuda_bf16.h>
#include <cuda_fp16.h>
#include <math.h>
#include <stdio.h>
#include <stdlib.h>
#include <string.h>
#include <vector>
#include "../../include/dasr_b200.h"

#define CK(x)                                                                      \
  do {                                                                             \
    cudaError_t e_ = (x);                                                          \
    if (e_ != cudaSuccess) {                                                       \
      printf("CUDA error %s at %s:%d\n", cudaGetErrorString(e_), __FILE__, __LINE__); \
      exit(2);                                                                     \
    }                                                                              \
  } while (0)

extern "C" int dasr_probe_mma_rate(int n, int sbo, int iters, int a_step, double* cycles_per_mma);
extern "C" int dasr_probe_tma_rate(int row_elems, int rows_per_box, int cs, int store, double* cycles_per_box);
extern "C" int dasr_probe_mma2_rate(int n, int iters, double* cycles_per_mma);
static unsigned long long rng_state = 0x1234567ULL;
static inline unsigned rnd() {
  rng_state = rng_state * 6364136223846793005ULL + 1442695040888963407ULL;
  return (unsigned)(rng_state >> 33);
}
static inline float rnd_q(int range, float denom) { return (float)((int)(rnd() % (2 * range + 1)) - range) / denom; }

static int g_fail = 0;
static void report(const char* name, double maxerr, double tol) {
  bool ok = maxerr <= tol;
  printf("[%s] %-58s max_err=%.3e tol=%.1e\n", ok ? "PASS" : "FAIL", name, maxerr, tol);
  if (!ok) g_fail++;
}

template <typename T> static T* dalloc(size_t n) { T* p; CK(cudaMalloc(&p, n * sizeof(T))); CK(cudaMemset(p, 0, n * sizeof(T))); return p; }
template <typename T> static void h2d(T* d, const std::vector<T>& h) { CK(cudaMemcpy(d, h.data(), h.size() * sizeof(T), cudaMemcpyHostToDevice)); }
template <typename T> static std::vector<T> d2h(const T* d, size_t n) { std::vector<T> h(n); CK(cudaMemcpy(h.data(), d, n * sizeof(T), cudaMemcpyDeviceToHost)); return h; }

static void cpu_conv(const std::vector<float>& in, int N, int H, int W, int cin, int in_cs, int in_coff,
                     const std::vector<float>& w, const std::vector<float>* bias, int cout, int kh, int kw, int stride,
                     int pad, int ups, int OH, int OW, std::vector<double>& out) {
  out.assign((size_t)N * OH * OW * cout, 0.0);
  for (int n = 0; n < N; n++)
    for (int oy = 0; oy < OH; oy++)
      for (int ox = 0; ox < OW; ox++)
        for (int co = 0; co < cout; co++) {
          double s = bias ? (*bias)[co] : 0.0;
          for (int dy = 0; dy < kh; dy++)
            for (int dx = 0; dx < kw; dx++) {
              int ty = oy * stride - pad + dy, tx = ox * stride - pad + dx;
              if (ty < 0 || tx < 0 || ty >= H * ups || tx >= W * ups) continue;
              int iy = ty / ups, ix = tx / ups;
              for (int ci = 0; ci < cin; ci++)
                s += (double)in[((size_t)(n * H + iy) * W + ix) * in_cs + in_coff + ci] *
                     (double)w[((size_t)(co * cin + ci) * kh + dy) * kw + dx];
            }
          out[((size_t)(n * OH + oy) * OW + ox) * cout + co] = s;
        }
}

static int g_math = 0;
static void test_f32(int N, int H, int W, int cin, int cout, int k, int stride, int pad, int ups) {
  char name[160];
  int in_cs = cin + 8, in_coff = 4;
  int OH = (H * ups + 2 * pad - k) / stride + 1, OW = (W * ups + 2 * pad - k) / stride + 1;
  std::vector<float> in((size_t)N * H * W * in_cs), w((size_t)cout * cin * k * k), b(cout);
  for (auto& v : in) v = rnd_q(8, 8.f);
  for (auto& v : w) v = rnd_q(8, 16.f);
  for (auto& v : b) v = rnd_q(8, 8.f);
  std::vector<double> ref;
  cpu_conv(in, N, H, W, cin, in_cs, in_coff, w, &b, cout, k, k, stride, pad, ups, OH, OW, ref);
  float *din = dalloc<float>(in.size()), *dw = dalloc<float>(w.size()), *dwp = dalloc<float>(w.size()),
        *db = dalloc<float>(cout), *dout = dalloc<float>(ref.size());
  h2d(din, in); h2d(dw, w); h2d(db, b);
  DasrConvF32Params p;
  memset(&p, 0, sizeof(p));
  p.math = g_math;
  p.N = N; p.H = H; p.W = W; p.cin = cin; p.in_cs = in_cs; p.in_coff = in_coff; p.OH = OH; p.OW = OW;
  p.cout = cout; p.out_cs = cout; p.out_coff = 0; p.kh = k; p.kw = k; p.stride = stride; p.pad = pad; p.ups = ups;
  p.mode = DASR_CONV_FWD; p.act = DASR_ACT_NONE; p.alpha = 1.f;
  int rc = dasr_pack_filter_f32(dw, dwp, cout, cin, k, k, 0, 0);
  rc |= dasr_conv2d_f32(din, dwp, db, nullptr, nullptr, dout, &p, 0);
  CK(cudaDeviceSynchronize());
  if (rc) printf("  rc=%d err=%s\n", rc, dasr_last_error());
  auto got = d2h(dout, ref.size());
  double me = 0;
  for (size_t i = 0; i < ref.size(); i++) me = fmax(me, fabs(got[i] - ref[i]));
  snprintf(name, sizeof(name), "conv_f32%s fwd N%d %dx%d cin%d cout%d k%d s%d p%d ups%d", g_math == 2 ? " tf32" : g_math == 3 ? " tf32x3" : "", N, H, W, cin, cout, k, stride, pad, ups);
  report(name, me, 1e-4);

  if (ups == 1) {
    std::vector<float> dy((size_t)N * OH * OW * cout);
    for (auto& v : dy) v = rnd_q(8, 8.f);
    std::vector<double> dxref((size_t)N * H * W * cin, 0.0);
    for (int n = 0; n < N; n++)
      for (int oy = 0; oy < OH; oy++)
        for (int ox = 0; ox < OW; ox++)
          for (int co = 0; co < cout; co++) {
            double g = dy[((size_t)(n * OH + oy) * OW + ox) * cout + co];
            for (int dyy = 0; dyy < k; dyy++)
              for (int dxx = 0; dxx < k; dxx++) {
                int iy = oy * stride - pad + dyy, ix = ox * stride - pad + dxx;
                if (iy < 0 || ix < 0 || iy >= H || ix >= W) continue;
                for (int ci = 0; ci < cin; ci++)
                  dxref[((size_t)(n * H + iy) * W + ix) * cin + ci] += g * w[((size_t)(co * cin + ci) * k + dyy) * k + dxx];
              }
          }
    float *ddy = dalloc<float>(dy.size()), *ddx = dalloc<float>(dxref.size()), *dwd = dalloc<float>(w.size());
    h2d(ddy, dy);
    DasrConvF32Params q;
    memset(&q, 0, sizeof(q));
  q.math = g_math;
    q.N = N; q.H = OH; q.W = OW; q.cin = cout; q.in_cs = cout; q.in_coff = 0; q.OH = H; q.OW = W; q.cout = cin;
    q.out_cs = cin; q.out_coff = 0; q.kh = k; q.kw = k; q.stride = stride; q.pad = pad; q.ups = 1;
    q.mode = DASR_CONV_DGRAD; q.alpha = 1.f;
    rc = dasr_pack_filter_f32(dw, dwd, cout, cin, k, k, 1, 0);
    rc |= dasr_conv2d_f32(ddy, dwd, nullptr, nullptr, nullptr, ddx, &q, 0);
    CK(cudaDeviceSynchronize());
    if (rc) printf("  rc=%d err=%s\n", rc, dasr_last_error());
    auto gx = d2h(ddx, dxref.size());
    me = 0;
    for (size_t i = 0; i < dxref.size(); i++) me = fmax(me, fabs(gx[i] - dxref[i]));
    snprintf(name, sizeof(name), "conv_f32%s dgrad N%d %dx%d cin%d cout%d k%d s%d p%d", g_math == 2 ? " tf32" : g_math == 3 ? " tf32x3" : "", N, H, W, cin, cout, k, stride, pad);
    report(name, me, 1e-4);

    std::vector<double> dwref(w.size(), 0.0), dbref(cout, 0.0);
    for (int n = 0; n < N; n++)
      for (int oy = 0; oy < OH; oy++)
        for (int ox = 0; ox < OW; ox++)
          for (int co = 0; co < cout; co++) {
            double g = dy[((size_t)(n * OH + oy) * OW + ox) * cout + co];
            dbref[co] += g;
            for (int dyy = 0; dyy < k; dyy++)
              for (int dxx = 0; dxx < k; dxx++) {
                int iy = oy * stride - pad + dyy, ix = ox * stride - pad + dxx;
                if (iy < 0 || ix < 0 || iy >= H || ix >= W) continue;
                for (int ci = 0; ci < cin; ci++)
                  dwref[((size_t)(co * cin + ci) * k + dyy) * k + dxx] +=
                      g * in[((size_t)(n * H + iy) * W + ix) * in_cs + in_coff + ci];
              }
          }
    size_t wsb = dasr_conv2d_wgrad_f32_workspace(&p);
    void* ws; CK(cudaMalloc(&ws, wsb));
    float *ddw = dalloc<float>(w.size()), *ddb = dalloc<float>(cout);
    rc = dasr_conv2d_wgrad_f32(din, ddy, ddw, ddb, &p, 0, ws, wsb, 0);
    CK(cudaDeviceSynchronize());
    if (rc) printf("  rc=%d err=%s\n", rc, dasr_last_error());
    auto gw = d2h(ddw, w.size());
    auto gb = d2h(ddb, (size_t)cout);
    me = 0;
    for (size_t i = 0; i < w.size(); i++) me = fmax(me, fabs(gw[i] - dwref[i]));
    for (int i = 0; i < cout; i++) me = fmax(me, fabs(gb[i] - dbref[i]));
    snprintf(name, sizeof(name), "conv_f32%s wgrad N%d %dx%d cin%d cout%d k%d s%d p%d", g_math == 2 ? " tf32" : g_math == 3 ? " tf32x3" : "", N, H, W, cin, cout, k, stride, pad);
    report(name, me, 2e-3);
    cudaFree(ddy); cudaFree(ddx); cudaFree(dwd); cudaFree(ws); cudaFree(ddw); cudaFree(ddb);
  }
  cudaFree(din); cudaFree(dw); cudaFree(dwp); cudaFree(db); cudaFree(dout);
}

static std::vector<__nv_bfloat16> to_bf16(const std::vector<float>& v) {
  std::vector<__nv_bfloat16> o(v.size());
  for (size_t i = 0; i < v.size(); i++) o[i] = __float2bfloat16(v[i]);
  return o;
}
static int g_f16 = 0;
static int g_tile_rev = 0;
static int g_up_staged = 0;
static std::vector<__nv_bfloat16> to_h16(const std::vector<float>& v) {
  if (!g_f16) return to_bf16(v);
  std::vector<__nv_bfloat16> o(v.size());
  for (size_t i = 0; i < v.size(); i++) {
    __half h = __float2half_rn(v[i]);
    memcpy(&o[i], &h, 2);
  }
  return o;
}
static inline float h16_to_float(__nv_bfloat16 x) {
  if (!g_f16) return __bfloat162float(x);
  __half h;
  memcpy(&h, &x, 2);
  return __half2float(h);
}

static void test_tc(int N, int H, int W, int cin, int cout, int nt, int kind, int a_mode, int epi) {
  char name[200];
  const int gk = (kind == 1) ? cout : cin;
  const int gn = (kind == 1) ? cin : cout;
  const int in_cs = gk + 32, in_coff = 8;
  const int mul = (kind == 2) ? 2 : 1;
  const int OH = H * mul, OW = W * mul;
  const int out_cs = gn + 16, out_coff = 8;
  std::vector<float> in((size_t)N * H * W * in_cs), w((size_t)cout * cin * 9), b(gn);
  for (auto& v : in) v = rnd_q(8, 8.f);
  for (auto& v : w) v = rnd_q(4, 16.f);
  for (auto& v : b) v = rnd_q(8, 8.f);
  std::vector<float> wref;
  if (kind == 1) {
    wref.assign((size_t)gn * gk * 9, 0.f);
    for (int kco = 0; kco < cout; kco++)
      for (int nci = 0; nci < cin; nci++)
        for (int t = 0; t < 9; t++) wref[((size_t)nci * gk + kco) * 9 + t] = w[((size_t)kco * cin + nci) * 9 + (8 - t)];
  } else {
    wref = w;
  }
  std::vector<double> ref;
  cpu_conv(in, N, H, W, gk, in_cs, in_coff, wref, &b, gn, 3, 3, 1, 1, mul, OH, OW, ref);
  std::vector<float> res1((size_t)N * OH * OW * gn), msk((size_t)N * OH * OW * gn);
  for (auto& v : res1) v = rnd_q(8, 8.f);
  for (auto& v : msk) v = rnd_q(8, 8.f);
  const float slope = 0.25f, alpha = 0.5f, mslope = 0.25f;
  const float beta1 = ((epi == 2 || epi == 5) && gn > 96) ? 0.f : 2.f;
  const int mc0 = gn >= 32 ? gn - 24 : 0, mc1 = gn;
  const int act_cols = (epi == 2 || epi == 4 || epi == 5) ? 16 * ((gn / 16 + 1) / 2) : gn;
  const float beta2 = (gn > 96) ? 0.f : -0.5f;
  if (epi == 1)
    for (size_t i = 0; i < ref.size(); i++) {
      double v = ref[i];
      v = v > 0 ? v : v * slope;
      v = alpha * v + beta1 * res1[i];
      int c = (int)(i % gn);
      if (c >= mc0 && c < mc1 && !(msk[i] > 0.f)) v *= mslope;
      ref[i] = v;
    }
  if (epi == 2 || epi == 5)
    for (size_t i = 0; i < ref.size(); i++) {
      int c = (int)(i % gn);
      double v = ref[i] + msk[i];
      if (c < act_cols) v = v > 0 ? v : v * slope;
      ref[i] = alpha * v + beta1 * res1[i] + beta2 * res1[(i + gn) % ref.size()];
    }
  if (epi == 7)
    for (size_t i = 0; i < ref.size(); i++) {
      int c = (int)(i % gn);
      double v = ref[i] + msk[i];
      if (c >= gn - 32 && !(res1[i] > 0.f)) v *= mslope;
      ref[i] = v;
    }
  if (epi == 4)
    for (size_t i = 0; i < ref.size(); i++) {
      int c = (int)(i % gn);
      double v = ref[i];
      const int ac = 16 * ((gn / 16 + 1) / 2);
      if (c < ac) v = v > 0 ? v : v * slope;
      ref[i] = alpha * v;
    }
  auto in_b = to_h16(in);
  auto res_b = to_h16(res1);
  auto msk_b = to_h16(msk);
  __nv_bfloat16* din = dalloc<__nv_bfloat16>(in_b.size());
  __nv_bfloat16* dres = dalloc<__nv_bfloat16>(res_b.size());
  __nv_bfloat16* dmsk = dalloc<__nv_bfloat16>(msk_b.size());
  __nv_bfloat16* dout = dalloc<__nv_bfloat16>((size_t)N * OH * OW * out_cs);
  float *dw = dalloc<float>(w.size()), *db = dalloc<float>(gn);
  size_t wpb = dasr_pack_filter_tc_bytes(cout, cin, kind);
  void* dwp; CK(cudaMalloc(&dwp, wpb));
  h2d(din, in_b); h2d(dres, res_b); h2d(dmsk, msk_b); h2d(dw, w); h2d(db, b);
  DasrConvTcParams p;
  memset(&p, 0, sizeof(p));
  int rc = dasr_conv_tc_setup(&p, kind);
  p.N = N; p.H = H; p.W = W; p.cin = gk; p.in_cs = in_cs; p.in_coff = in_coff;
  p.cout = gn; p.out_cs = out_cs; p.out_coff = out_coff; p.nt = nt;
  p.act = (epi == 1 || epi == 2 || epi >= 4) ? DASR_ACT_LRELU : DASR_ACT_NONE; p.slope = slope; p.alpha = (epi == 1 || epi == 2 || epi >= 4) ? alpha : 1.f;
  p.act_cols = act_cols;
  p.beta1 = beta1; p.res1_cs = gn; p.res1_coff = 0;
  p.beta2 = beta2; p.res2_cs = gn; p.res2_coff = 0;
  p.pre_cs = gn; p.pre_coff = 0;
  p.mask_cs = gn; p.mask_coff = mc0; p.mask_c0 = mc0; p.mask_c1 = mc1; p.mask_slope = mslope;
  p.a_mode = a_mode;
  p.f16 = g_f16;
  p.tile_rev = (epi == 4 || epi == 5 || epi == 7) ? g_tile_rev : 0;
  p.epi_mode = ((kind == 2 && !g_up_staged) || epi == 1 || nt % 32) ? 1 : 0;
  float* dnchw = nullptr;
  if (epi == 3) { p.epi_mode = 2; p.out_nc = 3; dnchw = dalloc<float>((size_t)N * 3 * OH * OW); }
  int pack_kind = kind;
  if (epi == 6) {
    rc |= dasr_conv_tc_setup(&p, 3);
    p.cout = 32; p.nt = 32; p.out_cs = 32; p.out_coff = 0; p.act_cols = 0;
    p.epi_mode = 3; p.out_nc = gn; pack_kind = 3; p.act = DASR_ACT_NONE; p.alpha = 1.f;
    dnchw = dalloc<float>((size_t)N * 3 * OH * OW);
    cudaFree(db); db = dalloc<float>(32); h2d(db, b);
    cudaFree(dwp); CK(cudaMalloc(&dwp, dasr_pack_filter_tc_bytes(cout, cin, 3)));
  }
  rc |= dasr_pack_filter_tc(dw, dwp, cout, cin, pack_kind | (g_f16 ? DASR_TC_PACK_F16 : 0), 0);
  __nv_bfloat16* dres2 = nullptr;
  if ((epi == 2 || epi == 5) && gn <= 96) {
    std::vector<__nv_bfloat16> r2(res_b.size());
    for (size_t i = 0; i < r2.size(); i++) r2[i] = res_b[(i + gn) % r2.size()];
    dres2 = dalloc<__nv_bfloat16>(r2.size());
    h2d(dres2, r2);
  }
  if (epi == 4 || epi == 5) p.mask_c0 = p.mask_c1 = 0;
  if (epi == 7) {
    p.act = DASR_ACT_NONE; p.alpha = 1.f; p.act_cols = 0; p.beta1 = 0.f; p.beta2 = 0.f;
    p.mask_c0 = gn - 32; p.mask_c1 = gn;
    rc |= dasr_conv_tc2(din, dwp, db, dmsk, dres, nullptr, dout, &p, 0);
  } else if (epi == 4)
    rc |= dasr_conv_tc2(din, dwp, db, nullptr, nullptr, nullptr, dout, &p, 0);
  else if (epi == 5)
    rc |= dasr_conv_tc2(din, dwp, db, dmsk, gn <= 96 ? dres : nullptr, dres2, dout, &p, 0);
  else
    rc |= dasr_conv_tc(din, dwp, db, epi == 2 ? dmsk : nullptr, (epi == 1 || (epi == 2 && gn <= 96)) ? dres : nullptr, dres2,
                       epi == 1 ? dmsk : nullptr, (epi == 3 || epi == 6) ? (void*)dnchw : (void*)dout, &p, 0);
  cudaError_t e = cudaDeviceSynchronize();
  snprintf(name, sizeof(name), "conv_tc%s kind%d amode%d N%d %dx%d K%d N%d nt%d epi%d mode%d", g_f16 ? " f16" : "", kind, a_mode, N, H, W, gk, gn, nt, epi, p.epi_mode);
  if (rc == DASR_E_SMEM && e == cudaSuccess) {
    printf("[SKIP] %s (does not fit shared memory in this A mode)\n", name);
    return;
  }
  if (rc || e != cudaSuccess) {
    printf("[FAIL] %s rc=%d err=%s cuda=%s\n", name, rc, dasr_last_error(), cudaGetErrorString(e));
    g_fail++;
    if (e != cudaSuccess) exit(3);
    return;
  }
  double me = 0, mref = 0;
  if (epi == 3 || epi == 6) {
    auto gotf = d2h(dnchw, (size_t)N * 3 * OH * OW);
    const int nch = (epi == 6) ? gn : 3;
    for (int n = 0; n < N; n++)
      for (int c = 0; c < nch; c++)
        for (size_t pp = 0; pp < (size_t)OH * OW; pp++) {
          double r = ref[((size_t)n * OH * OW + pp) * gn + c];
          double g = gotf[((size_t)n * nch + c) * OH * OW + pp];
          me = fmax(me, fabs(g - r) / (1.0 + fabs(r)));
        }
    report(name, me, 1e-5);
    cudaFree(dnchw);
  } else {
    auto got = d2h(dout, (size_t)N * OH * OW * out_cs);
    for (size_t pix = 0; pix < (size_t)N * OH * OW; pix++) {
      for (int c = 0; c < out_coff; c++) me = fmax(me, fabs(h16_to_float(got[pix * out_cs + c])));
      for (int c = out_coff + gn; c < out_cs; c++) me = fmax(me, fabs(h16_to_float(got[pix * out_cs + c])));
      for (int c = 0; c < gn; c++) {
        double r = ref[pix * gn + c];
        double g = h16_to_float(got[pix * out_cs + out_coff + c]);
        me = fmax(me, fabs(g - r) / (1.0 + fabs(r)));
        mref = fmax(mref, fabs(r));
      }
    }
    report(name, me, g_f16 ? 1e-3 : 8e-3);
  }
  if (dres2) cudaFree(dres2);
  cudaFree(din); cudaFree(dres); cudaFree(dmsk); cudaFree(dout); cudaFree(dw); cudaFree(db); cudaFree(dwp);
}

static void test_wgrad_tc(int N, int H, int W, int cin, int cout) {
  char name[160];
  const int x_cs = cin + 32, x_coff = 8, dy_cs = cout + 16, dy_coff = 8;
  std::vector<float> x((size_t)N * H * W * x_cs), dy((size_t)N * H * W * dy_cs);
  for (auto& v : x) v = rnd_q(8, 8.f);
  for (auto& v : dy) v = rnd_q(8, 8.f);
  std::vector<double> ref((size_t)cout * cin * 9, 0.0);
  for (int n = 0; n < N; n++)
    for (int oy = 0; oy < H; oy++)
      for (int ox = 0; ox < W; ox++)
        for (int t = 0; t < 9; t++) {
          int iy = oy - 1 + t / 3, ix = ox - 1 + t % 3;
          if (iy < 0 || ix < 0 || iy >= H || ix >= W) continue;
          const float* xp = &x[((size_t)(n * H + iy) * W + ix) * x_cs + x_coff];
          const float* gp = &dy[((size_t)(n * H + oy) * W + ox) * dy_cs + dy_coff];
          for (int co = 0; co < cout; co++) {
            double g = gp[co];
            if (g == 0.0) continue;
            for (int ci = 0; ci < cin; ci++) ref[((size_t)co * cin + ci) * 9 + t] += g * xp[ci];
          }
        }
  auto xb = to_bf16(x), dyb = to_bf16(dy);
  __nv_bfloat16 *dx = dalloc<__nv_bfloat16>(xb.size()), *ddy = dalloc<__nv_bfloat16>(dyb.size());
  h2d(dx, xb); h2d(ddy, dyb);
  float* dw = dalloc<float>(ref.size());
  size_t wsb = dasr_conv3x3_wgrad_tc_workspace(N, H, W, cin, cout);
  void* ws; CK(cudaMalloc(&ws, wsb));
  int rc = dasr_conv3x3_wgrad_tc(dx, x_cs, x_coff, ddy, dy_cs, dy_coff, dw, N, H, W, cin, cout, 0, ws, wsb, 0);
  cudaError_t e = cudaDeviceSynchronize();
  snprintf(name, sizeof(name), "wgrad_tc N%d %dx%d cin%d cout%d", N, H, W, cin, cout);
  if (rc || e != cudaSuccess) {
    printf("[FAIL] %s rc=%d err=%s cuda=%s\n", name, rc, dasr_last_error(), cudaGetErrorString(e));
    g_fail++;
    if (e != cudaSuccess) exit(3);
    return;
  }
  auto got = d2h(dw, ref.size());
  double me = 0;
  for (size_t i = 0; i < ref.size(); i++) me = fmax(me, fabs(got[i] - ref[i]));
  report(name, me, 1e-3);
  cudaFree(dx); cudaFree(ddy); cudaFree(dw); cudaFree(ws);
}

static void bench_tc(int N, int H, int W, int cin, int cout, int nt, int kind, int a_mode, int iters) {
  const int in_cs = 192;
  const int mul = (kind == 2) ? 2 : 1;
  size_t in_n = (size_t)N * H * W * in_cs, out_n = (size_t)N * H * mul * W * mul * in_cs;
  __nv_bfloat16* din = dalloc<__nv_bfloat16>(in_n);
  __nv_bfloat16* dout = dalloc<__nv_bfloat16>(out_n);
  std::vector<float> w((size_t)cout * cin * 9);
  for (auto& v : w) v = rnd_q(4, 64.f);
  float *dw = dalloc<float>(w.size()), *db = dalloc<float>(256);
  h2d(dw, w);
  void* dwp; CK(cudaMalloc(&dwp, dasr_pack_filter_tc_bytes(cout, cin, kind)));
  DasrConvTcParams p;
  memset(&p, 0, sizeof(p));
  dasr_conv_tc_setup(&p, kind);
  p.N = N; p.H = H; p.W = W; p.cin = cin; p.in_cs = in_cs; p.in_coff = 0;
  p.cout = cout; p.out_cs = in_cs; p.out_coff = (cout <= 128) ? 64 : 0; p.nt = nt;
  p.act = DASR_ACT_LRELU; p.slope = 0.2f; p.alpha = 1.f; p.a_mode = a_mode; p.act_cols = cout;
  p.epi_mode = (kind == 2 || nt % 32) ? 1 : 0;
  if (kind == 1) dasr_pack_filter_tc(dw, dwp, cin, cout, kind, 0);
  else dasr_pack_filter_tc(dw, dwp, cout, cin, kind, 0);
  int rc = 0;
  for (int i = 0; i < 3; i++) rc |= dasr_conv_tc(din, dwp, db, nullptr, nullptr, nullptr, nullptr, dout, &p, 0);
  cudaError_t e = cudaDeviceSynchronize();
  if (rc || e != cudaSuccess) {
    printf("bench conv_tc cin%d cout%d nt%d kind%d amode%d: rc=%d %s cuda=%s\n", cin, cout, nt, kind, a_mode, rc,
           dasr_last_error(), cudaGetErrorString(e));
    if (e != cudaSuccess) exit(3);
    return;
  }
  cudaEvent_t e0, e1;
  cudaEventCreate(&e0); cudaEventCreate(&e1);
  cudaEventRecord(e0);
  for (int i = 0; i < iters; i++) dasr_conv_tc(din, dwp, db, nullptr, nullptr, nullptr, nullptr, dout, &p, 0);
  cudaEventRecord(e1);
  CK(cudaEventSynchronize(e1));
  float ms; cudaEventElapsedTime(&ms, e0, e1);
  ms /= iters;
  double taps = (kind == 2) ? 9.0 : 9.0;
  double flops = 2.0 * N * H * mul * W * mul * cin * cout * taps;
  printf("bench conv_tc kind%d amode%d %dx%dx%d cin%-3d cout%-3d nt%-3d : %8.3f ms  %7.1f TFLOP/s (algorithmic)\n", kind,
         a_mode, N, H, W, cin, cout, nt, ms, flops / ms * 1e-9);
  cudaFree(din); cudaFree(dout); cudaFree(dw); cudaFree(db); cudaFree(dwp);
}

static void bench_tc_fused(int N, int H, int W, int cin, int cout, int nt, int with_pre, int iters, int in_cs = 0, int out_cs = 0,
                           int pair = 0) {
  const int cs = 256;
  const bool planar = in_cs > 0;
  size_t n = (size_t)N * H * W * (planar ? in_cs : cs);
  __nv_bfloat16* buf = dalloc<__nv_bfloat16>(n);
  __nv_bfloat16* obuf = planar ? dalloc<__nv_bfloat16>((size_t)N * H * W * out_cs) : buf;
  std::vector<float> w((size_t)cout * cin * 9);
  for (auto& v : w) v = rnd_q(4, 64.f);
  float* dw = dalloc<float>(w.size());
  h2d(dw, w);
  void* dwp; CK(cudaMalloc(&dwp, dasr_pack_filter_tc_bytes(cout, cin, 0)));
  DasrConvTcParams p;
  memset(&p, 0, sizeof(p));
  dasr_conv_tc_setup(&p, 0);
  p.N = N; p.H = H; p.W = W; p.cin = cin; p.in_cs = planar ? in_cs : cs; p.in_coff = 0;
  p.cout = cout; p.out_cs = planar ? out_cs : cs; p.out_coff = planar ? 0 : cs - cout; p.nt = nt;
  p.act = DASR_ACT_LRELU; p.slope = 0.2f; p.alpha = 1.f; p.act_cols = 32; p.epi_mode = 0;
  p.pre_cs = p.out_cs; p.pre_coff = p.out_coff;
  if (getenv("EPI1") && !with_pre) p.epi_mode = 1;
  dasr_pack_filter_tc(dw, dwp, cout, cin, 0, 0);
  void* pre = with_pre ? (void*)obuf : nullptr;
  int rc = 0;
  auto run = [&]() {
    return pair ? dasr_conv_tc2(buf, dwp, nullptr, pre, nullptr, nullptr, obuf, &p, 0)
                : dasr_conv_tc(buf, dwp, nullptr, pre, nullptr, nullptr, nullptr, obuf, &p, 0);
  };
  for (int i = 0; i < 3; i++) rc |= run();
  cudaError_t e = cudaDeviceSynchronize();
  if (rc || e != cudaSuccess) {
    printf("bench fused cin%d cout%d nt%d: rc=%d %s cuda=%s\n", cin, cout, nt, rc, dasr_last_error(), cudaGetErrorString(e));
    if (e != cudaSuccess) exit(3);
    return;
  }
  cudaEvent_t e0, e1;
  cudaEventCreate(&e0); cudaEventCreate(&e1);
  cudaEventRecord(e0);
  for (int i = 0; i < iters; i++) run();
  cudaEventRecord(e1);
  CK(cudaEventSynchronize(e1));
  float ms; cudaEventElapsedTime(&ms, e0, e1);
  ms /= iters;
  double tiles_per_sm = (double)N * (H / 16) * (W / 8) / 148.0 * (cout / nt);
  if (pair) tiles_per_sm = (double)N * (H / 16) * (W / 8) / 148.0;
  printf("bench fused  %dx%dx%d K%-3d N%-3d nt%-3d pre%d %s%s: %8.3f ms  %7.1f TFLOP/s  %6.2f us/tile\n", N, H, W, cin, cout, nt,
         with_pre, planar ? "planar " : "", pair ? "pair " : "", ms, 2.0 * N * H * W * cin * cout * 9 / ms * 1e-9, ms * 1e3 / tiles_per_sm);
  if (planar) cudaFree(obuf);
  cudaFree(buf); cudaFree(dw); cudaFree(dwp);
}

static void bench_f32(int N, int H, int W, int cin, int cout, int iters) {
  size_t in_n = (size_t)N * H * W * cin, out_n = (size_t)N * H * W * cout;
  float *din = dalloc<float>(in_n), *dout = dalloc<float>(out_n), *dw = dalloc<float>((size_t)9 * cin * cout), *db = dalloc<float>(cout);
  DasrConvF32Params p;
  memset(&p, 0, sizeof(p));
  p.N = N; p.H = H; p.W = W; p.cin = cin; p.in_cs = cin; p.OH = H; p.OW = W; p.cout = cout; p.out_cs = cout;
  p.kh = p.kw = 3; p.stride = 1; p.pad = 1; p.ups = 1; p.alpha = 1.f;
  for (int i = 0; i < 2; i++) dasr_conv2d_f32(din, dw, db, nullptr, nullptr, dout, &p, 0);
  CK(cudaDeviceSynchronize());
  cudaEvent_t e0, e1;
  cudaEventCreate(&e0); cudaEventCreate(&e1);
  cudaEventRecord(e0);
  for (int i = 0; i < iters; i++) dasr_conv2d_f32(din, dw, db, nullptr, nullptr, dout, &p, 0);
  cudaEventRecord(e1);
  CK(cudaEventSynchronize(e1));
  float ms; cudaEventElapsedTime(&ms, e0, e1);
  ms /= iters;
  printf("bench conv_f32 %dx%dx%d cin%-3d cout%-3d : %8.3f ms  %7.2f TFLOP/s\n", N, H, W, cin, cout, ms,
         2.0 * N * H * W * cin * cout * 9 / ms * 1e-9);
  cudaFree(din); cudaFree(dout); cudaFree(dw); cudaFree(db);
}

int main(int argc, char** argv) {
  bool do_check = argc == 1, do_bench = argc == 1;
  for (int i = 1; i < argc; i++) {
    if (!strcmp(argv[i], "check")) do_check = true;
    if (!strcmp(argv[i], "bench")) do_bench = true;
    if (!strcmp(argv[i], "tmarate")) {
      for (int store = 0; store <= 1; store++)
        for (int re : {32, 64, 128, 256})
          for (int cs : {256, 0}) {
            const int rows = 128;
            if ((long)re * 2 * rows > 49152) continue;
            const int pitch = cs ? cs : re;
            double c = 0;
            int rc = dasr_probe_tma_rate(re, rows, pitch, store, &c);
            printf("tma_%s row=%4d B rows/box=%3d pitch=%4d B : %8.1f cycles/box  %6.2f cycles/row  %6.2f B/clk/SM rc=%d\n",
                   store ? "store" : "load ", re * 2, rows, pitch * 2, c, c / rows, re * 2.0 * rows / c, rc);
          }
      return 0;
    }
    if (!strcmp(argv[i], "mmarate")) {
      int ns[] = {32, 64, 96, 128, 192, 256};
      for (int nowait = 0; nowait <= 1; nowait++)
        for (int nacc : {1, 2, 4})
          for (int n : ns) {
            if (n * nacc > 512) continue;
            double c = 0;
            int rc = dasr_probe_mma_rate(n, 640, 200, 64 | (nacc << 16) | (nowait << 20), &c);
            printf("mma_rate M128 N%-3d K16 accumulators=%d %s : %7.1f cycles/MMA  (N/2=%d) rc=%d\n", n, nacc,
                   nowait ? "back-to-back" : "wait/18     ", c, n / 2, rc);
          }
      return 0;
    }
    if (!strcmp(argv[i], "mma2rate")) {
      for (int n : {64, 96, 128, 160, 192, 256}) {
        double c = 0;
        int rc = dasr_probe_mma2_rate(n, 200, &c);
        printf("mma2_rate M256 N%-3d K16 cta_group::2 back-to-back : %7.1f cycles/MMA  (%.1f per 128-pixel tile) rc=%d %s\n", n, c, c / 2,
               rc, rc ? dasr_last_error() : "");
      }
      return 0;
    }
    if (!strcmp(argv[i], "fused")) {
      bench_tc_fused(16, 256, 256, 64, 192, 96, 0, 10);
      bench_tc_fused(16, 256, 256, 32, 160, 160, 1, 10);
      bench_tc_fused(16, 256, 256, 32, 160, 160, 0, 10);
      bench_tc_fused(16, 256, 256, 32, 128, 128, 1, 10);
      bench_tc_fused(16, 256, 256, 32, 96, 96, 1, 10);
      bench_tc_fused(16, 256, 256, 32, 64, 64, 1, 10);
      bench_tc_fused(16, 256, 256, 32, 64, 64, 0, 10);
      bench_tc_fused(2, 256, 256, 32, 64, 64, 1, 40);
      bench_tc_fused(2, 256, 256, 32, 64, 64, 0, 40);
      bench_tc_fused(16, 256, 256, 64, 64, 64, 1, 10);
      bench_tc_fused(16, 256, 256, 64, 64, 64, 0, 10);
      bench_tc_fused(2, 256, 256, 64, 64, 64, 0, 40);
      bench_tc_fused(16, 256, 256, 32, 64, 64, 1, 10, 32, 64);
      bench_tc_fused(16, 256, 256, 32, 64, 64, 0, 10, 32, 64);
      bench_tc_fused(16, 256, 256, 64, 64, 64, 1, 10, 64, 64);
      bench_tc_fused(16, 256, 256, 32, 128, 128, 1, 10, 32, 128);
      bench_tc_fused(16, 256, 256, 64, 192, 96, 0, 10, 64, 192);
      bench_tc_fused(16, 256, 256, 64, 192, 192, 0, 10, 0, 0, 1);
      bench_tc_fused(16, 256, 256, 64, 192, 192, 0, 10, 64, 192, 1);
      bench_tc_fused(16, 256, 256, 32, 128, 128, 0, 10, 0, 0, 1);
      bench_tc_fused(16, 256, 256, 32, 64, 64, 1, 10, 0, 0, 1);
      bench_tc_fused(16, 256, 256, 32, 64, 64, 0, 10, 0, 0, 1);
      bench_tc_fused(16, 256, 256, 64, 64, 64, 1, 10, 0, 0, 1);
      bench_tc_fused(16, 256, 256, 96, 64, 64, 1, 10, 0, 0, 1);
      bench_tc_fused(16, 256, 256, 96, 128, 128, 1, 10, 0, 0, 1);
      bench_tc_fused(16, 256, 256, 64, 128, 128, 1, 10, 0, 0, 1);
      bench_tc_fused(16, 256, 256, 32, 32, 32, 1, 10, 0, 0, 1);
      bench_tc_fused(16, 256, 256, 32, 32, 32, 1, 10, 0, 0, 0);
      bench_tc_fused(16, 256, 256, 128, 64, 64, 1, 10, 0, 0, 1);
      return 0;
    }
    if (!strcmp(argv[i], "prof")) {
      bench_tc(16, 256, 256, 64, 32, 32, 0, 0, 1);
      bench_tc(16, 256, 256, 160, 32, 32, 0, 0, 1);
      bench_tc(16, 256, 256, 32, 192, 192, 1, 0, 1);
      return 0;
    }
  }
  setvbuf(stdout, NULL, _IOLBF, 0);
  cudaDeviceProp prop;
  CK(cudaGetDeviceProperties(&prop, 0));
  printf("device: %s sm_%d%d SMs=%d smem_optin=%zu\n", prop.name, prop.major, prop.minor, prop.multiProcessorCount,
         prop.sharedMemPerBlockOptin);
  if (do_check) {
    for (g_math = 0; g_math <= 3; g_math = g_math ? g_math + 1 : 2) {
      test_f32(2, 9, 11, 3, 64, 3, 1, 1, 1);
      test_f32(2, 8, 8, 32, 32, 3, 1, 1, 1);
      test_f32(1, 7, 5, 64, 3, 3, 1, 1, 1);
      test_f32(2, 12, 10, 9, 64, 4, 2, 1, 1);
      test_f32(1, 9, 9, 16, 20, 4, 1, 1, 1);
      test_f32(1, 6, 7, 16, 16, 3, 1, 1, 2);
      test_f32(1, 8, 8, 8, 1, 4, 1, 1, 1);
      test_f32(1, 10, 10, 12, 8, 5, 1, 2, 1);
      test_f32(2, 16, 16, 64, 128, 4, 2, 1, 1);
      test_f32(2, 9, 9, 64, 1, 4, 1, 1, 1);
      test_f32(1, 11, 7, 30, 2, 3, 1, 1, 1);
    }
    g_math = 0;
    test_wgrad_tc(1, 16, 8, 32, 32);
    test_wgrad_tc(1, 16, 8, 64, 32);
    test_wgrad_tc(2, 20, 13, 96, 32);
    test_wgrad_tc(3, 32, 24, 160, 32);
    test_wgrad_tc(2, 32, 16, 192, 64);
    test_wgrad_tc(1, 48, 40, 64, 64);
    for (int am = 1; am >= 0; am--) {
      test_tc(1, 16, 8, 32, 32, 32, 0, am, 0);
      test_tc(2, 32, 32, 64, 32, 32, 0, am, 0);
      test_tc(1, 20, 13, 96, 32, 32, 0, am, 1);
      test_tc(2, 32, 24, 192, 64, 32, 0, am, 1);
      test_tc(1, 32, 16, 64, 64, 64, 0, am, 1);
      test_tc(1, 20, 13, 96, 32, 32, 0, am, 2);
      test_tc(2, 24, 16, 64, 64, 64, 0, am, 2);
      test_tc(1, 40, 24, 32, 160, 160, 0, am, 2);
      test_tc(1, 19, 11, 64, 192, 96, 0, am, 2);
      test_tc(1, 21, 10, 64, 16, 16, 0, am, 3);
      if (am == 0) {
        test_tc(1, 21, 10, 64, 3, 32, 0, am, 6);
        test_tc(2, 32, 24, 64, 3, 32, 0, am, 6);
        test_tc(1, 16, 8, 32, 1, 32, 0, am, 6);
      }
      test_tc(1, 24, 24, 160, 32, 160, 1, am, 1);
      test_tc(1, 16, 16, 192, 64, 96, 1, am, 0);
      if (am == 0) {
        test_tc(1, 16, 8, 64, 192, 192, 0, 0, 4);
        test_tc(1, 19, 11, 64, 192, 192, 0, 0, 4);
        test_tc(2, 32, 16, 64, 192, 192, 0, 0, 4);
        test_tc(4, 96, 64, 64, 192, 192, 0, 0, 4);
        test_tc(1, 24, 16, 32, 128, 128, 0, 0, 4);
        test_tc(1, 16, 16, 192, 64, 192, 1, 0, 4);
        test_tc(1, 20, 13, 96, 64, 64, 0, 0, 5);
        test_tc(3, 48, 40, 64, 64, 64, 0, 0, 5);
        test_tc(2, 40, 24, 32, 128, 128, 0, 0, 5);
        test_tc(1, 32, 24, 64, 192, 192, 0, 0, 5);
        test_tc(4, 96, 64, 32, 64, 64, 0, 0, 5);
        test_tc(2, 40, 24, 32, 32, 32, 0, 0, 5);
        test_tc(1, 20, 13, 32, 96, 96, 0, 0, 5);
        test_tc(2, 32, 24, 32, 160, 160, 0, 0, 5);
        test_tc(1, 19, 11, 64, 96, 96, 0, 0, 4);
        test_tc(2, 24, 16, 160, 32, 160, 1, 0, 7);
        test_tc(1, 20, 13, 128, 32, 128, 1, 0, 7);
        test_tc(2, 32, 24, 96, 32, 96, 1, 0, 7);
        test_tc(1, 19, 11, 192, 64, 192, 1, 0, 7);
        g_tile_rev = 1;
        test_tc(1, 19, 11, 64, 192, 192, 0, 0, 4);
        test_tc(4, 96, 64, 64, 192, 192, 0, 0, 4);
        test_tc(3, 48, 40, 64, 64, 64, 0, 0, 5);
        test_tc(1, 20, 13, 32, 96, 96, 0, 0, 5);
        g_tile_rev = 0;
        test_tc(1, 16, 8, 64, 128, 64, 0, 0, 4);
        test_tc(2, 24, 16, 64, 128, 32, 0, 0, 5);
        test_tc(1, 20, 13, 96, 192, 96, 0, 0, 4);
        test_tc(1, 16, 16, 512, 64, 32, 0, 0, 4);
        test_tc(1, 16, 16, 128, 64, 64, 1, 0, 4);
        g_f16 = 1;
        test_tc(2, 32, 16, 64, 192, 192, 0, 0, 4);
        test_tc(1, 20, 13, 96, 64, 64, 0, 0, 5);
        test_tc(2, 40, 24, 32, 32, 32, 0, 0, 5);
        test_tc(2, 32, 24, 32, 160, 160, 0, 0, 5);
        test_tc(1, 20, 13, 96, 32, 32, 0, 0, 2);
        test_tc(1, 16, 16, 64, 64, 64, 2, 0, 0);
        test_tc(1, 21, 10, 64, 16, 16, 0, 0, 3);
        g_f16 = 0;
      }
      test_tc(1, 16, 16, 64, 64, 64, 2, am, 1);
      if (am == 0) {
        g_up_staged = 1;
        test_tc(1, 16, 16, 64, 64, 64, 2, am, 0);
        test_tc(2, 19, 9, 64, 64, 64, 2, am, 0);
        test_tc(1, 20, 13, 32, 96, 96, 2, am, 0);
        g_up_staged = 0;
      }
      test_tc(2, 19, 9, 64, 64, 32, 2, am, 0);
    }
  }
  if (do_bench) {
    const int N = 16, H = 256, W = 256;
    for (int am = 0; am <= 1; am++) {
      bench_tc(N, H, W, 64, 32, 32, 0, am, 10);
      bench_tc(N, H, W, 96, 32, 32, 0, am, 10);
      bench_tc(N, H, W, 128, 32, 32, 0, am, 10);
      bench_tc(N, H, W, 160, 32, 32, 0, am, 10);
      bench_tc(N, H, W, 192, 64, 32, 0, am, 10);
      bench_tc(N, H, W, 64, 64, 64, 0, am, 10);
    }
    bench_tc(N, H, W, 192, 64, 64, 0, 0, 10);
    bench_tc(N, H, W, 64, 64, 64, 2, 0, 5);
    bench_tc(N, H, W, 32, 192, 192, 1, 0, 10);
    bench_f32(4, 256, 256, 64, 64, 3);
    bench_f32(4, 256, 256, 192, 64, 3);
  }
  printf("selftest done: %d failure(s)\n", g_fail);
  return g_fail ? 1 : 0;
}
```

Baseline: 374.4.

## Load epilogue residuals via direct global loads and allow 64-channel A-tile TMA loads

The tc2 conv kernel drops the TMA-staged pre/residual shared-memory buffers and their barriers. Epilogue warps now fetch pre-activation and residual operands directly from global memory with __ldcg before waiting on the accumulator, which frees shared memory and removes the extra TMA traffic. The producer can also load 64-channel A chunks per stage when chunk64 is set, halving the number of TMA loads and barrier round-trips, with the MMA descriptors adjusted for the wider rows and swizzle. A TMA/cp.async mixing probe and new chunk-list self-tests are added. The risk is uncoalesced or exposed global-load latency in the epilogue.

```diff
diff --git a/dasr_b200/csrc/conv_tc.cu b/dasr_b200/csrc/conv_tc.cu
--- a/dasr_b200/csrc/conv_tc.cu
+++ b/dasr_b200/csrc/conv_tc.cu
@@ -1,4 +1,5 @@
 #include <stdlib.h>
+#include <vector>
 #include "tc_common.cuh"
 
 namespace dasr {
@@ -685,6 +686,76 @@
   }
 }
 
+__global__ void __launch_bounds__(64, 1) tma_mix_kernel(const __grid_constant__ CUtensorMap ld, const __grid_constant__ CUtensorMap st,
+                                                        int nld, uint32_t ld_bytes, int nst, int cpa_rows, int cpa_row_b,
+                                                        const uint8_t* g, int cs, int iters, long long* out) {
+  extern __shared__ __align__(1024) uint8_t smem_raw[];
+  uint8_t* smem = reinterpret_cast<uint8_t*>((reinterpret_cast<uintptr_t>(smem_raw) + 1023) & ~uintptr_t(1023));
+  uint8_t* sLd = smem;
+  uint8_t* sSt = smem + 4 * 24576;
+  uint8_t* sCp = sSt + 16384;
+  __shared__ uint64_t bar[4];
+  if (threadIdx.x == 0) {
+    for (int i = 0; i < 4; i++) mbar_init(&bar[i], 1);
+    fence_barrier_init();
+  }
+  __syncthreads();
+  auto tile = [&](int i, int salt, int& x0, int& y0, int& n) {
+    const uint32_t t = (uint32_t)(((long)blockIdx.x * 7919 + (long)i * 104729 + salt) % 8192);
+    x0 = (int)(t & 31) * 8;
+    y0 = (int)((t >> 5) & 15) * 16;
+    n = (int)(t >> 9);
+  };
+  const long long t0 = clock64();
+  if (threadIdx.x == 0) {
+    uint32_t ph[4] = {0, 0, 0, 0};
+    int k = 0;
+    for (int i = 0; i < iters; i++) {
+      for (int j = 0; j < nld; j++, k++) {
+        const int s = k & 3;
+        if (k >= 4) { mbar_wait(&bar[s], ph[s]); ph[s] ^= 1; }
+        int x0, y0, n;
+        tile(k, 0, x0, y0, n);
+        mbar_expect_tx(&bar[s], ld_bytes);
+        tma_load_4d(sLd + s * 24576, &ld, &bar[s], 0, x0 - 1, y0 - 1, n);
+      }
+      for (int j = 0; j < nst; j++) {
+        int x0, y0, n;
+        tile(i * nst + j, 4099, x0, y0, n);
+        tma_store_4d(&st, sSt, 128, x0, y0, n);
+        bulk_commit();
+        asm volatile("cp.async.bulk.wait_group.read 2;" ::: "memory");
+      }
+    }
+    for (int s = 0; s < 4 && s < k; s++) {
+      const int kk = k - 1 - s;
+      mbar_wait(&bar[kk & 3], ph[kk & 3]);
+    }
+    bulk_wait0();
+    out[2 * blockIdx.x] = clock64() - t0;
+  } else if (threadIdx.x >= 32 && cpa_rows > 0) {
+    const int lane = threadIdx.x - 32;
+    const int cpr = cpa_row_b / 16;
+    const int nchunk = cpa_rows * cpr;
+    for (int i = 0; i < iters; i++) {
+      int x0, y0, n;
+      tile(i, 8191, x0, y0, n);
+      const uint32_t dst = smem_u32(sCp + (i % 3) * 16384);
+      for (int c = lane; c < nchunk; c += 32) {
+        const int r = c / cpr, q = c - r * cpr;
+        const long pix = ((long)n * 256 + y0 + (r >> 3)) * 256 + x0 + (r & 7);
+        asm volatile("cp.async.cg.shared.global [%0], [%1], 16;" ::"r"(dst + (uint32_t)(r * cpa_row_b + q * 16)),
+                     "l"(g + pix * cs * 2 + 128 + q * 16) : "memory");
+      }
+      asm volatile("cp.async.commit_group;" ::: "memory");
+      asm volatile("cp.async.wait_group 2;" ::: "memory");
+    }
+    asm volatile("cp.async.wait_group 0;" ::: "memory");
+    __syncwarp();
+    if (lane == 0) out[2 * blockIdx.x + 1] = clock64() - t0;
+  }
+}
+
 }
 
 using namespace dasr;
@@ -1006,4 +1077,48 @@
   return DASR_OK;
 }
 
-}
+int dasr_probe_tma_mix(int ld_c, int ld_halo, int nld, int st_c, int nst, int cpa_c, int iters, double* cyc_tma, double* cyc_cpa) {
+  PFN_encodeTiled enc = get_encode();
+  if (!enc) return DASR_E_NODRIVER;
+  const int cs = 256, NI = 32;
+  const size_t bytes = (size_t)NI * 256 * 256 * cs * 2;
+  void* buf;
+  if (cudaMalloc(&buf, bytes) != cudaSuccess) return DASR_E_LAUNCH;
+  cudaMemset(buf, 0, bytes);
+  CUtensorMap tl, ts;
+  auto make = [&](CUtensorMap* m, int c, int bw, int bh) {
+    cuuint64_t gdim[4] = {(cuuint64_t)cs, 256, 256, (cuuint64_t)NI};
+    cuuint64_t gstr[3] = {(cuuint64_t)cs * 2, (cuuint64_t)256 * cs * 2, (cuuint64_t)256 * 256 * cs * 2};
+    cuuint32_t box[4] = {(cuuint32_t)c, (cuuint32_t)bw, (cuuint32_t)bh, 1};
+    cuuint32_t estr[4] = {1, 1, 1, 1};
+    return enc(m, CU_TENSOR_MAP_DATA_TYPE_BFLOAT16, 4, buf, gdim, gstr, box, estr, CU_TENSOR_MAP_INTERLEAVE_NONE,
+               c == 64 ? CU_TENSOR_MAP_SWIZZLE_128B : CU_TENSOR_MAP_SWIZZLE_64B,
+               c == 64 ? CU_TENSOR_MAP_L2_PROMOTION_L2_128B : CU_TENSOR_MAP_L2_PROMOTION_L2_64B, CU_TENSOR_MAP_FLOAT_OOB_FILL_NONE);
+  };
+  const int lc = ld_c ? ld_c : 32, sc = st_c ? st_c : 32;
+  if (make(&tl, lc, ld_halo ? 10 : 8, ld_halo ? 18 : 16) != CUDA_SUCCESS || make(&ts, sc, 8, 16) != CUDA_SUCCESS) {
+    cudaFree(buf);
+    set_error("probe tma mix: encode");
+    return DASR_E_LAUNCH;
+  }
+  const int nsm = num_sms();
+  long long* d;
+  cudaMalloc(&d, (size_t)2 * nsm * 8);
+  cudaMemset(d, 0, (size_t)2 * nsm * 8);
+  const uint32_t ld_bytes = (uint32_t)lc * 2 * (ld_halo ? 180 : 128);
+  cudaFuncSetAttribute(tma_mix_kernel, cudaFuncAttributeMaxDynamicSharedMemorySize, 200 * 1024);
+  tma_mix_kernel<<<nsm, 64, 200 * 1024>>>(tl, ts, ld_c ? nld : 0, ld_bytes, st_c ? nst : 0, cpa_c ? 128 : 0, cpa_c * 2,
+                                          (const uint8_t*)buf, cs, iters, d);
+  std::vector<long long> h((size_t)2 * nsm);
+  cudaError_t e = cudaMemcpy(h.data(), d, (size_t)2 * nsm * 8, cudaMemcpyDeviceToHost);
+  cudaFree(d);
+  cudaFree(buf);
+  if (e != cudaSuccess) { set_error("probe tma mix: %s", cudaGetErrorString(e)); return DASR_E_LAUNCH; }
+  double s0 = 0, s1 = 0;
+  for (int i = 0; i < nsm; i++) { s0 += (double)h[2 * i]; s1 += (double)h[2 * i + 1]; }
+  *cyc_tma = s0 / nsm / iters;
+  *cyc_cpa = s1 / nsm / iters;
+  return DASR_OK;
+}
+
+}
diff --git a/dasr_b200/csrc/conv_tc2.cu b/dasr_b200/csrc/conv_tc2.cu
--- a/dasr_b200/csrc/conv_tc2.cu
+++ b/dasr_b200/csrc/conv_tc2.cu
@@ -10,13 +10,18 @@
 constexpr int TC2_MAX_BLOCKS = 6;
 
 struct Tc2Maps {
-  CUtensorMap m[8];
+  CUtensorMap m[2];
 };
 
 struct Tc2Args {
   DasrConvTcParams p;
   const float* bias;
+  const uint8_t* pre;
+  const uint8_t* res1;
+  const uint8_t* res2;
   int nchunks;
+  int chunk64;
+  int nloads;
   int n_half;
   int tiles_x, tiles_y;
   long ntiles;
@@ -36,9 +41,7 @@
   uint8_t* sW = smem;
   uint8_t* sA = smem + a.w_bytes;
   uint8_t* sS = sA + (size_t)a.stages * a.a_stage_bytes;
-  uint8_t* sR1 = sS + (size_t)a.nblk * EPI_BLK64_BYTES;
-  uint8_t* sR2 = sR1 + (NRES >= 1 ? (size_t)a.nblk * EPI_BLK64_BYTES : 0);
-  uint64_t* bars = reinterpret_cast<uint64_t*>(sR2 + (NRES >= 2 ? (size_t)a.nblk * EPI_BLK64_BYTES : 0));
+  uint64_t* bars = reinterpret_cast<uint64_t*>(sS + (size_t)a.nblk * EPI_BLK64_BYTES);
   constexpr bool HAS_LOADS = HAS_PRE || NRES > 0;
   uint64_t* full_bar = bars;
   uint64_t* empty_bar = bars + TC2_MAX_STAGES;
@@ -47,8 +50,7 @@
   uint64_t* tempty_bar = tfull_bar + 2;
   uint64_t* sfull_bar = tempty_bar + 2;
   uint64_t* sfree_bar = sfull_bar + TC2_MAX_BLOCKS;
-  uint64_t* pre_bar = sfree_bar + TC2_MAX_BLOCKS;
-  uint32_t* tmem_ptr = reinterpret_cast<uint32_t*>(pre_bar + TC2_MAX_BLOCKS);
+  uint32_t* tmem_ptr = reinterpret_cast<uint32_t*>(sfree_bar + TC2_MAX_BLOCKS);
   float* sBias = reinterpret_cast<float*>(bars + 40);
 
   const DasrConvTcParams& p = a.p;
@@ -74,7 +76,6 @@
     for (int b = 0; b < a.nblk; b++) {
       mbar_init(&sfull_bar[b], TC2_EPI_WARPS);
       mbar_init(&sfree_bar[b], 1);
-      mbar_init(&pre_bar[b], 1);
     }
     fence_barrier_init();
   }
@@ -116,9 +117,10 @@
       for (long it = 0; it < niter; it++) {
         int x0, y0, n;
         tile_of(it, x0, y0, n);
-        for (int c = 0; c < a.nchunks; c++) {
+        for (int l = 0; l < a.nloads; l++) {
+          const int c = a.chunk64 ? 2 * l : l;
           mbar_wait(&empty_bar[stage], phase ^ 1);
-          if (rank == 0) mbar_expect_tx(&full_bar[stage], 2u * A_HALO_BYTES);
+          if (rank == 0) mbar_expect_tx(&full_bar[stage], 2u * (uint32_t)((a.chunk64 ? 2 : 1) * A_HALO_BYTES));
           tma2_load_4d(sA + (size_t)stage * a.a_stage_bytes, &tmap_in, &full_bar[stage],
                        p.nchunk_list ? p.chunk_off[c] : p.in_coff + c * CHUNK, x0 - 1, y0 - 1, n);
           if (++stage == a.stages) { stage = 0; phase ^= 1; }
@@ -129,8 +131,9 @@
   } else if (warp == 1) {
     if (rank == 0) {
       const uint32_t idesc = make_idesc_16(256, cout, p.f16);
-      const uint32_t a_sbo = (uint32_t)(HALO_W * ROW_B);
-      const uint64_t a_hi = ((uint64_t)((a_sbo >> 4) & 0x3FFF) << 32) | ((uint64_t)1 << 46) | ((uint64_t)4 << 61) | ((uint64_t)1 << 16);
+      const uint32_t a_row = a.chunk64 ? 2u * ROW_B : (uint32_t)ROW_B;
+      const uint32_t a_sbo = (uint32_t)HALO_W * a_row;
+      const uint64_t a_hi = ((uint64_t)((a_sbo >> 4) & 0x3FFF) << 32) | ((uint64_t)1 << 46) | ((uint64_t)(a.chunk64 ? 2 : 4) << 61) | ((uint64_t)1 << 16);
       const uint64_t b_hi = ((uint64_t)(((8 * ROW_B) >> 4) & 0x3FFF) << 32) | ((uint64_t)1 << 46) | ((uint64_t)4 << 61) | ((uint64_t)1 << 16);
       const uint32_t a_lo0 = smem_u32(sA) >> 4;
       const uint32_t a_stage_lo = (uint32_t)a.a_stage_bytes >> 4;
@@ -138,7 +141,8 @@
       const uint32_t b_slot_lo = (uint32_t)(a.n_half * ROW_B) >> 4;
       uint32_t tap_lo[9];
 #pragma unroll
-      for (int t = 0; t < 9; t++) tap_lo[t] = (uint32_t)(((t / 3) * HALO_W + (t % 3)) * ROW_B) >> 4;
+      for (int t = 0; t < 9; t++) tap_lo[t] = ((uint32_t)((t / 3) * HALO_W + (t % 3)) * a_row) >> 4;
+      const int halves = a.chunk64 ? 2 : 1;
       mbar_wait(w_bar, 0);
       tc_fence_after();
       int stage = 0;
@@ -148,22 +152,25 @@
         mbar_wait(&tempty_bar[acc], ((uint32_t)(it >> 1) & 1) ^ 1);
         tc_fence_after();
         const uint32_t d_tmem = tmem_base + (uint32_t)(acc * a.acc_stride);
-        for (int c = 0; c < a.nchunks; c++) {
+        for (int l = 0; l < a.nloads; l++) {
           mbar_wait(&full_bar[stage], phase);
           tc_fence_after();
           if (elect_one()) {
-            const uint32_t a_lo = a_lo0 + (uint32_t)stage * a_stage_lo;
-            uint32_t b_lo = b_lo0 + (uint32_t)c * b_slot_lo;
             const uint32_t b_tap_step = (uint32_t)a.nchunks * b_slot_lo;
-#pragma unroll
-            for (int tap = 0; tap < 9; tap++) {
-              const uint32_t al = a_lo + tap_lo[tap];
-              umma2_bf16(d_tmem, a_hi | (uint64_t)(al & 0x3FFF), b_hi | (uint64_t)(b_lo & 0x3FFF), idesc, (uint32_t)((c | tap) != 0));
-              umma2_bf16(d_tmem, a_hi | (uint64_t)((al + 2) & 0x3FFF), b_hi | (uint64_t)((b_lo + 2) & 0x3FFF), idesc, 1u);
-              b_lo += b_tap_step;
+            for (int h = 0; h < halves; h++) {
+              const int c = l * halves + h;
+              const uint32_t a_lo = a_lo0 + (uint32_t)stage * a_stage_lo + (uint32_t)h * 4u;
+              uint32_t b_lo = b_lo0 + (uint32_t)c * b_slot_lo;
+#pragma unroll
+              for (int tap = 0; tap < 9; tap++) {
+                const uint32_t al = a_lo + tap_lo[tap];
+                umma2_bf16(d_tmem, a_hi | (uint64_t)(al & 0x3FFF), b_hi | (uint64_t)(b_lo & 0x3FFF), idesc, (uint32_t)((c | tap) != 0));
+                umma2_bf16(d_tmem, a_hi | (uint64_t)((al + 2) & 0x3FFF), b_hi | (uint64_t)((b_lo + 2) & 0x3FFF), idesc, 1u);
+                b_lo += b_tap_step;
+              }
             }
             umma2_commit_mc(&empty_bar[stage]);
-            if (c == a.nchunks - 1) umma2_commit_mc(&tfull_bar[acc]);
+            if (l == a.nloads - 1) umma2_commit_mc(&tfull_bar[acc]);
           }
           __syncwarp();
           if (++stage == a.stages) { stage = 0; phase ^= 1; }
@@ -175,33 +182,7 @@
       pdl_wait();
       const uint32_t nb = (uint32_t)a.nb, nblk = (uint32_t)a.nblk;
       const uint32_t total = (uint32_t)niter * nb;
-      const uint32_t nld = (uint32_t)((HAS_PRE ? 1 : 0) + NRES);
-      const bool mask_mode = (NRES >= 1) && (p.mask_c1 > p.mask_c0);
-      auto issue_loads = [&](uint32_t k) {
-        const uint32_t b = k % nblk;
-        int x0, y0, n;
-        const uint32_t kt = k / nb;
-        tile_of((long)kt, x0, y0, n);
-        const int i = (int)(k - kt * nb);
-        const int wide = i < a.nb64 ? 1 : 0;
-        const int col = co_base + i * 64;
-        const bool need_r1 = !mask_mode || (col < p.mask_c1 && col + (wide ? 64 : 32) > p.mask_c0);
-        mbar_expect_tx(&pre_bar[b], (nld - (need_r1 ? 0u : 1u)) * (uint32_t)(wide ? EPI_BLK64_BYTES : EPI_BLK32_BYTES));
-        if constexpr (HAS_PRE) tma_load_4d(sS + (size_t)b * EPI_BLK64_BYTES, &em.m[wide ? 2 : 3], &pre_bar[b], p.pre_coff + col, x0, y0, n);
-        if constexpr (NRES >= 1) {
-          if (need_r1) tma_load_4d(sR1 + (size_t)b * EPI_BLK64_BYTES, &em.m[wide ? 4 : 5], &pre_bar[b], p.res1_coff + col, x0, y0, n);
-        }
-        if constexpr (NRES >= 2) tma_load_4d(sR2 + (size_t)b * EPI_BLK64_BYTES, &em.m[wide ? 6 : 7], &pre_bar[b], p.res2_coff + col, x0, y0, n);
-      };
-      if constexpr (HAS_LOADS)
-        for (uint32_t k = 0; k < nblk && k < total; k++) issue_loads(k);
-      auto retire = [&](uint32_t k) {
-        if constexpr (HAS_LOADS) {
-          if (k + nblk < total) issue_loads(k + nblk);
-        } else {
-          mbar_arrive(&sfree_bar[k % nblk]);
-        }
-      };
+      auto retire = [&](uint32_t k) { mbar_arrive(&sfree_bar[k % nblk]); };
       int x0 = 0, y0 = 0, n = 0;
       bool live = false;
       uint32_t i = 0;
@@ -233,28 +214,55 @@
     const int act = p.act, f16 = p.f16;
     const float slope = p.slope, alpha = p.alpha;
     const bool scale = alpha != 1.f;
-    const uint32_t sS_u = smem_u32(sS), sR1_u = smem_u32(sR1), sR2_u = smem_u32(sR2), sBias_u = smem_u32(sBias);
+    const uint32_t sS_u = smem_u32(sS), sBias_u = smem_u32(sBias);
     const bool has_bias = a.bias != nullptr;
+    const bool mask_mode = (NRES >= 1) && (p.mask_c1 > p.mask_c0);
+    if constexpr (HAS_LOADS) pdl_wait();
+    auto ld32 = [&](const uint8_t* base, int cs, int ch, long pix, uint4* d) {
+      if (pix < 0) {
+        d[0] = d[1] = make_uint4(0, 0, 0, 0);
+      } else {
+        const uint4* s = reinterpret_cast<const uint4*>(base + (pix * cs + ch) * 2);
+        d[0] = __ldcg(s);
+        d[1] = __ldcg(s + 1);
+      }
+    };
     uint32_t k = 0;
     for (long it = 0; it < niter; it++) {
       const int acc = (int)(it & 1);
-      mbar_wait(&tfull_bar[acc], (uint32_t)(it >> 1) & 1);
-      tc_fence_after();
+      long pix = -1;
+      if constexpr (HAS_LOADS) {
+        int x0, y0, n;
+        tile_of(it, x0, y0, n);
+        const int x = x0 + (m & 7), y = y0 + (m >> 3);
+        if (x < p.W && y < p.H && n < p.N) pix = ((long)n * p.H + y) * p.W + x;
+      }
       const uint32_t t_addr = tmem_base + ((uint32_t)(q * 32) << 16) + (uint32_t)(acc * a.acc_stride);
       for (int i = 0; i < a.nb; i++, k++) {
         const int b = (int)(k % (uint32_t)a.nblk);
-        if constexpr (HAS_LOADS) {
-          mbar_wait(&pre_bar[b], (k / (uint32_t)a.nblk) & 1);
-        } else {
-          if (k >= (uint32_t)a.nblk) mbar_wait(&sfree_bar[b], ((k / (uint32_t)a.nblk) & 1) ^ 1);
-        }
+        const int c0 = i * 64 + wg * 16, c1 = c0 + 32;
+        const int nh = i < a.nb64 ? 2 : 1;
+        uint4 pv[2][2], r1v[2][2], r2v[2][2];
+#pragma unroll
+        for (int h = 0; h < 2; h++) {
+          if (h < nh) {
+            const int co = co_base + (h ? c1 : c0);
+            if constexpr (HAS_PRE) ld32(a.pre, p.pre_cs, p.pre_coff + co, pix, pv[h]);
+            if constexpr (NRES >= 1) {
+              if (!mask_mode || (co >= p.mask_c0 && co < p.mask_c1)) ld32(a.res1, p.res1_cs, p.res1_coff + co, pix, r1v[h]);
+            }
+            if constexpr (NRES >= 2) ld32(a.res2, p.res2_cs, p.res2_coff + co, pix, r2v[h]);
+          }
+        }
+        if (i == 0) {
+          mbar_wait(&tfull_bar[acc], (uint32_t)(it >> 1) & 1);
+          tc_fence_after();
+        }
+        if (k >= (uint32_t)a.nblk) mbar_wait(&sfree_bar[b], ((k / (uint32_t)a.nblk) & 1) ^ 1);
         const bool wide = i < a.nb64;
         const uint32_t rowoff = (uint32_t)m * (wide ? 128u : 64u);
         const uint32_t bS = sS_u + (uint32_t)b * EPI_BLK64_BYTES + rowoff;
-        const uint32_t bR1 = sR1_u + (uint32_t)b * EPI_BLK64_BYTES + rowoff;
-        const uint32_t bR2 = sR2_u + (uint32_t)b * EPI_BLK64_BYTES + rowoff;
         uint32_t ra[16], rb[16];
-        const int c0 = i * 64 + wg * 16, c1 = c0 + 32;
         tmem_ld16(t_addr + c0, ra);
         if (wide) tmem_ld16(t_addr + c1, rb);
         tmem_ld_wait();
@@ -286,8 +294,8 @@
           const int sw = wide ? sw128 : sw64;
           const uint32_t o0 = (uint32_t)(((ch) ^ sw) << 4), o1 = (uint32_t)(((ch + 1) ^ sw) << 4);
           if constexpr (HAS_PRE) {
-            fma_h16x8(v, lds128(bS + o0), 1.f, f16);
-            fma_h16x8(v + 8, lds128(bS + o1), 1.f, f16);
+            fma_h16x8(v, pv[h][0], 1.f, f16);
+            fma_h16x8(v + 8, pv[h][1], 1.f, f16);
           }
           if (do_act) {
             if (act == DASR_ACT_LRELU) {
@@ -303,10 +311,10 @@
             for (int j = 0; j < 16; j++) v[j] *= alpha;
           }
           if constexpr (NRES >= 1) {
-            if (p.mask_c1 > p.mask_c0) {
+            if (mask_mode) {
               const int co = co_base + cg;
               if (co >= p.mask_c0 && co < p.mask_c1) {
-                const uint4 m0 = lds128(bR1 + o0), m1 = lds128(bR1 + o1);
+                const uint4 m0 = r1v[h][0], m1 = r1v[h][1];
                 const short* ms0 = reinterpret_cast<const short*>(&m0);
                 const short* ms1 = reinterpret_cast<const short*>(&m1);
 #pragma unroll
@@ -316,13 +324,13 @@
                 }
               }
             } else {
-              fma_h16x8(v, lds128(bR1 + o0), p.beta1, f16);
-              fma_h16x8(v + 8, lds128(bR1 + o1), p.beta1, f16);
+              fma_h16x8(v, r1v[h][0], p.beta1, f16);
+              fma_h16x8(v + 8, r1v[h][1], p.beta1, f16);
             }
           }
           if constexpr (NRES >= 2) {
-            fma_h16x8(v, lds128(bR2 + o0), p.beta2, f16);
-            fma_h16x8(v + 8, lds128(bR2 + o1), p.beta2, f16);
+            fma_h16x8(v, r2v[h][0], p.beta2, f16);
+            fma_h16x8(v + 8, r2v[h][1], p.beta2, f16);
           }
           uint4 o[2];
           pack_h16x16(v, o, f16);
@@ -392,13 +400,24 @@
 
 extern "C" {
 
-static int tc2_plan(const DasrConvTcParams* p, int has_pre, int nres, int* stages_out, int* nblk_out) {
+static int tc2_chunk64(const DasrConvTcParams* p) {
+  const int nchunks = p->cin / CHUNK;
+  if (nchunks % 2) return 0;
+  if (p->nchunk_list > 0)
+    for (int i = 0; i < nchunks; i += 2)
+      if (p->chunk_off[i + 1] != p->chunk_off[i] + CHUNK) return 0;
+  return 1;
+}
+
+static int tc2_a_stage_bytes(int chunk64) { return ((chunk64 ? 2 : 1) * A_HALO_BYTES + 1023) / 1024 * 1024; }
+
+static int tc2_plan(const DasrConvTcParams* p, int* stages_out, int* nblk_out) {
   const int nchunks = p->cin / CHUNK;
   const long w_bytes = (long)9 * nchunks * (p->nt / 2) * ROW_B;
-  const int a_stage = (A_HALO_BYTES + 1023) / 1024 * 1024;
+  const int kper = tc2_chunk64(p) ? 2 : 1;
+  const int a_stage = tc2_a_stage_bytes(kper == 2);
   const int bar_bytes = 40 * 8 + 256 * 4 + 64;
-  const int per_blk = (1 + nres) * EPI_BLK64_BYTES;
-  (void)has_pre;
+  const int per_blk = EPI_BLK64_BYTES;
   static int force_nblk = -1;
   if (force_nblk < 0) {
     const char* e = getenv("DASR_TC2_NBLK");
@@ -410,7 +429,7 @@
       const long avail = (long)SMEM_LIMIT - 1024 - w_bytes - (long)nblk * per_blk - bar_bytes;
       int stages = (int)(avail / a_stage);
       if (stages > TC2_MAX_STAGES) stages = TC2_MAX_STAGES;
-      if (stages >= want) {
+      if (stages >= 2 && stages * kper >= want) {
         *stages_out = stages;
         *nblk_out = nblk;
         return 1;
@@ -424,8 +443,7 @@
   if (p->nvar != 1 || p->ntaps != 9 || p->out_mul != 1 || p->epi_mode != 0 || p->a_mode != 0) return 0;
   if (p->nt % 32 != 0 || p->nt < 32 || p->nt > 256 || p->cout % p->nt != 0 || p->cin % CHUNK != 0 || p->cin <= 0) return 0;
   int st, nb;
-  const int nres = (p->res1_cs > 0 ? 1 : 0) + (p->res2_cs > 0 ? 1 : 0);
-  return tc2_plan(p, p->pre_cs > 0 ? 1 : 0, nres, &st, &nb);
+  return tc2_plan(p, &st, &nb);
 }
 
 int dasr_conv_tc2(const void* in, const void* w, const float* bias, const void* pre, const void* res1, const void* res2,
@@ -451,9 +469,9 @@
   if (p->mask_c1 > p->mask_c0)
     DASR_REQUIRE(res1 && !res2 && p->mask_c0 % 16 == 0 && p->mask_c1 % 16 == 0 && p->mask_c1 <= p->cout,
                  "conv_tc2: mask mode takes the activation as res1 (no res2) and a range of whole 16-channel groups");
-  if (pre) DASR_REQUIRE(p->pre_cs % 8 == 0 && p->pre_coff % 8 == 0 && p->pre_coff + p->cout <= p->pre_cs, "conv_tc2: pre slice");
-  if (res1) DASR_REQUIRE(p->res1_cs % 8 == 0 && p->res1_coff % 8 == 0 && p->res1_coff + p->cout <= p->res1_cs, "conv_tc2: res1 slice");
-  if (res2) DASR_REQUIRE(p->res2_cs % 8 == 0 && p->res2_coff % 8 == 0 && p->res2_coff + p->cout <= p->res2_cs, "conv_tc2: res2 slice");
+  if (pre) DASR_REQUIRE(((uintptr_t)pre & 15) == 0 && p->pre_cs % 8 == 0 && p->pre_coff % 8 == 0 && p->pre_coff + p->cout <= p->pre_cs, "conv_tc2: pre slice");
+  if (res1) DASR_REQUIRE(((uintptr_t)res1 & 15) == 0 && p->res1_cs % 8 == 0 && p->res1_coff % 8 == 0 && p->res1_coff + p->cout <= p->res1_cs, "conv_tc2: res1 slice");
+  if (res2) DASR_REQUIRE(((uintptr_t)res2 & 15) == 0 && p->res2_cs % 8 == 0 && p->res2_coff % 8 == 0 && p->res2_coff + p->cout <= p->res2_cs, "conv_tc2: res2 slice");
   PFN_encodeTiled enc = get_encode();
   if (!enc) {
     set_error("conv_tc2: cuTensorMapEncodeTiled not available");
@@ -463,25 +481,30 @@
   Tc2Args a;
   a.p = *p;
   a.bias = bias;
+  a.pre = static_cast<const uint8_t*>(pre);
+  a.res1 = static_cast<const uint8_t*>(res1);
+  a.res2 = static_cast<const uint8_t*>(res2);
   a.nchunks = p->cin / CHUNK;
+  a.chunk64 = tc2_chunk64(p);
+  a.nloads = a.chunk64 ? a.nchunks / 2 : a.nchunks;
   a.n_half = p->nt / 2;
   a.tiles_x = cdiv(p->W, TILE_W);
   a.tiles_y = cdiv(p->H, TILE_H);
   a.ntiles = (long)p->N * a.tiles_x * a.tiles_y;
   a.w_bytes = 9 * a.nchunks * a.n_half * ROW_B;
-  a.a_stage_bytes = (A_HALO_BYTES + 1023) / 1024 * 1024;
+  a.a_stage_bytes = tc2_a_stage_bytes(a.chunk64);
   a.nb64 = p->nt / 64;
   a.nb = a.nb64 + ((p->nt & 32) ? 1 : 0);
   a.acc_stride = 256;
   const int bar_bytes = 40 * 8 + 256 * 4 + 64;
   int stages = 0, nblk = 0;
-  if (!tc2_plan(p, has_pre, nres, &stages, &nblk)) {
-    set_error("conv_tc2: filters (%d B per CTA) + %d epilogue block arrays do not fit shared memory", a.w_bytes, 1 + nres);
+  if (!tc2_plan(p, &stages, &nblk)) {
+    set_error("conv_tc2: filters (%d B per CTA) + the epilogue block ring do not fit shared memory", a.w_bytes);
     return DASR_E_SMEM;
   }
   a.stages = stages;
   a.nblk = nblk;
-  size_t smem = 1024 + (size_t)a.w_bytes + (size_t)stages * a.a_stage_bytes + (size_t)nblk * (1 + nres) * EPI_BLK64_BYTES + bar_bytes;
+  size_t smem = 1024 + (size_t)a.w_bytes + (size_t)stages * a.a_stage_bytes + (size_t)nblk * EPI_BLK64_BYTES + bar_bytes;
   if (smem < 120 * 1024) smem = 120 * 1024;
 
   CUtensorMap tm_in, tm_w;
@@ -489,11 +512,11 @@
   {
     cuuint64_t gdim[4] = {(cuuint64_t)p->in_cs, (cuuint64_t)p->W, (cuuint64_t)p->H, (cuuint64_t)p->N};
     cuuint64_t gstr[3] = {(cuuint64_t)p->in_cs * 2, (cuuint64_t)p->W * p->in_cs * 2, (cuuint64_t)p->H * p->W * p->in_cs * 2};
-    cuuint32_t box[4] = {CHUNK, HALO_W, HALO_H, 1};
+    cuuint32_t box[4] = {(cuuint32_t)(a.chunk64 ? 2 * CHUNK : CHUNK), HALO_W, HALO_H, 1};
     cuuint32_t estr[4] = {1, 1, 1, 1};
     CUresult r = enc(&tm_in, CU_TENSOR_MAP_DATA_TYPE_BFLOAT16, 4, const_cast<void*>(in), gdim, gstr, box, estr,
-                     CU_TENSOR_MAP_INTERLEAVE_NONE, CU_TENSOR_MAP_SWIZZLE_64B,
-                     p->in_cs > CHUNK ? CU_TENSOR_MAP_L2_PROMOTION_L2_64B : CU_TENSOR_MAP_L2_PROMOTION_L2_128B,
+                     CU_TENSOR_MAP_INTERLEAVE_NONE, a.chunk64 ? CU_TENSOR_MAP_SWIZZLE_128B : CU_TENSOR_MAP_SWIZZLE_64B,
+                     (p->in_cs > CHUNK && !a.chunk64) ? CU_TENSOR_MAP_L2_PROMOTION_L2_64B : CU_TENSOR_MAP_L2_PROMOTION_L2_128B,
                      CU_TENSOR_MAP_FLOAT_OOB_FILL_NONE);
     if (r != CUDA_SUCCESS) { set_error("conv_tc2: cuTensorMapEncodeTiled(input) failed: %d", (int)r); return DASR_E_LAUNCH; }
   }
@@ -508,27 +531,19 @@
                      CU_TENSOR_MAP_FLOAT_OOB_FILL_NONE);
     if (r != CUDA_SUCCESS) { set_error("conv_tc2: cuTensorMapEncodeTiled(filter) failed: %d", (int)r); return DASR_E_LAUNCH; }
   }
-  {
-    const void* bases[4] = {out, pre, res1, res2};
-    const int css[4] = {p->out_cs, p->pre_cs, p->res1_cs, p->res2_cs};
-    const char* names[4] = {"output", "pre", "res1", "res2"};
-    for (int t = 0; t < 4; t++) {
-      em.m[2 * t] = em.m[2 * t + 1] = tm_in;
-      if (!bases[t]) continue;
-      for (int narrow = 0; narrow < 2; narrow++) {
-        if (narrow ? !(p->nt & 32) : (a.nb64 == 0)) continue;
-        const int width = narrow ? 32 : 64;
-        cuuint64_t gdim[4] = {(cuuint64_t)css[t], (cuuint64_t)p->W, (cuuint64_t)p->H, (cuuint64_t)p->N};
-        cuuint64_t gstr[3] = {(cuuint64_t)css[t] * 2, (cuuint64_t)p->W * css[t] * 2, (cuuint64_t)p->H * p->W * css[t] * 2};
-        cuuint32_t box[4] = {(cuuint32_t)width, TILE_W, TILE_H, 1};
-        cuuint32_t estr[4] = {1, 1, 1, 1};
-        CUresult r = enc(&em.m[2 * t + narrow], CU_TENSOR_MAP_DATA_TYPE_BFLOAT16, 4, const_cast<void*>(bases[t]), gdim, gstr, box, estr,
-                         CU_TENSOR_MAP_INTERLEAVE_NONE, narrow ? CU_TENSOR_MAP_SWIZZLE_64B : CU_TENSOR_MAP_SWIZZLE_128B,
-                         (narrow && css[t] > 32) ? CU_TENSOR_MAP_L2_PROMOTION_L2_64B : CU_TENSOR_MAP_L2_PROMOTION_L2_128B,
-                         CU_TENSOR_MAP_FLOAT_OOB_FILL_NONE);
-        if (r != CUDA_SUCCESS) { set_error("conv_tc2: cuTensorMapEncodeTiled(%s) failed: %d", names[t], (int)r); return DASR_E_LAUNCH; }
-      }
-    }
+  for (int narrow = 0; narrow < 2; narrow++) {
+    em.m[narrow] = tm_in;
+    if (narrow ? !(p->nt & 32) : (a.nb64 == 0)) continue;
+    const int width = narrow ? 32 : 64;
+    cuuint64_t gdim[4] = {(cuuint64_t)p->out_cs, (cuuint64_t)p->W, (cuuint64_t)p->H, (cuuint64_t)p->N};
+    cuuint64_t gstr[3] = {(cuuint64_t)p->out_cs * 2, (cuuint64_t)p->W * p->out_cs * 2, (cuuint64_t)p->H * p->W * p->out_cs * 2};
+    cuuint32_t box[4] = {(cuuint32_t)width, TILE_W, TILE_H, 1};
+    cuuint32_t estr[4] = {1, 1, 1, 1};
+    CUresult r = enc(&em.m[narrow], CU_TENSOR_MAP_DATA_TYPE_BFLOAT16, 4, out, gdim, gstr, box, estr,
+                     CU_TENSOR_MAP_INTERLEAVE_NONE, narrow ? CU_TENSOR_MAP_SWIZZLE_64B : CU_TENSOR_MAP_SWIZZLE_128B,
+                     (narrow && p->out_cs > 32) ? CU_TENSOR_MAP_L2_PROMOTION_L2_64B : CU_TENSOR_MAP_L2_PROMOTION_L2_128B,
+                     CU_TENSOR_MAP_FLOAT_OOB_FILL_NONE);
+    if (r != CUDA_SUCCESS) { set_error("conv_tc2: cuTensorMapEncodeTiled(output) failed: %d", (int)r); return DASR_E_LAUNCH; }
   }
   typedef void (*KernelFn)(const CUtensorMap, const CUtensorMap, const Tc2Maps, const Tc2Args);
   static const KernelFn kernels[6] = {conv_tc2_kernel<false, 0>, conv_tc2_kernel<false, 1>, conv_tc2_kernel<false, 2>,
diff --git a/dasr_b200/csrc/selftest.cu b/dasr_b200/csrc/selftest.cu
--- a/dasr_b200/csrc/selftest.cu
+++ b/dasr_b200/csrc/selftest.cu
@@ -20,6 +20,8 @@
 extern "C" int dasr_probe_mma_rate(int n, int sbo, int iters, int a_step, double* cycles_per_mma);
 extern "C" int dasr_probe_tma_rate(int row_elems, int rows_per_box, int cs, int store, double* cycles_per_box);
 extern "C" int dasr_probe_mma2_rate(int n, int iters, double* cycles_per_mma);
+extern "C" int dasr_probe_tma_mix(int ld_c, int ld_halo, int nld, int st_c, int nst, int cpa_c, int iters, double* cyc_tma,
+                                  double* cyc_cpa);
 static unsigned long long rng_state = 0x1234567ULL;
 static inline unsigned rnd() {
   rng_state = rng_state * 6364136223846793005ULL + 1442695040888963407ULL;
@@ -167,6 +169,7 @@
 static int g_f16 = 0;
 static int g_tile_rev = 0;
 static int g_up_staged = 0;
+static int g_chunks = 0;
 static std::vector<__nv_bfloat16> to_h16(const std::vector<float>& v) {
   if (!g_f16) return to_bf16(v);
   std::vector<__nv_bfloat16> o(v.size());
@@ -187,7 +190,10 @@
   char name[200];
   const int gk = (kind == 1) ? cout : cin;
   const int gn = (kind == 1) ? cin : cout;
-  const int in_cs = gk + 32, in_coff = 8;
+  const int in_cs = gk + 32 + (g_chunks == 2 ? 32 : 0), in_coff = 8;
+  const int nchl = g_chunks ? gk / 32 : 0;
+  int chunk_off[8] = {0};
+  for (int c = 0; c < nchl; c++) chunk_off[c] = in_coff + 32 * c + (g_chunks == 2 && c >= 1 ? 32 : 0);
   const int mul = (kind == 2) ? 2 : 1;
   const int OH = H * mul, OW = W * mul;
   const int out_cs = gn + 16, out_coff = 8;
@@ -205,7 +211,14 @@
     wref = w;
   }
   std::vector<double> ref;
-  cpu_conv(in, N, H, W, gk, in_cs, in_coff, wref, &b, gn, 3, 3, 1, 1, mul, OH, OW, ref);
+  if (nchl) {
+    std::vector<float> g((size_t)N * H * W * gk);
+    for (size_t pix = 0; pix < (size_t)N * H * W; pix++)
+      for (int ci = 0; ci < gk; ci++) g[pix * gk + ci] = in[pix * in_cs + chunk_off[ci / 32] + ci % 32];
+    cpu_conv(g, N, H, W, gk, gk, 0, wref, &b, gn, 3, 3, 1, 1, mul, OH, OW, ref);
+  } else {
+    cpu_conv(in, N, H, W, gk, in_cs, in_coff, wref, &b, gn, 3, 3, 1, 1, mul, OH, OW, ref);
+  }
   std::vector<float> res1((size_t)N * OH * OW * gn), msk((size_t)N * OH * OW * gn);
   for (auto& v : res1) v = rnd_q(8, 8.f);
   for (auto& v : msk) v = rnd_q(8, 8.f);
@@ -270,6 +283,8 @@
   p.a_mode = a_mode;
   p.f16 = g_f16;
   p.tile_rev = (epi == 4 || epi == 5 || epi == 7) ? g_tile_rev : 0;
+  p.nchunk_list = nchl;
+  for (int c = 0; c < nchl; c++) p.chunk_off[c] = chunk_off[c];
   p.epi_mode = ((kind == 2 && !g_up_staged) || epi == 1 || nt % 32) ? 1 : 0;
   float* dnchw = nullptr;
   if (epi == 3) { p.epi_mode = 2; p.out_nc = 3; dnchw = dalloc<float>((size_t)N * 3 * OH * OW); }
@@ -303,7 +318,8 @@
     rc |= dasr_conv_tc(din, dwp, db, epi == 2 ? dmsk : nullptr, (epi == 1 || (epi == 2 && gn <= 96)) ? dres : nullptr, dres2,
                        epi == 1 ? dmsk : nullptr, (epi == 3 || epi == 6) ? (void*)dnchw : (void*)dout, &p, 0);
   cudaError_t e = cudaDeviceSynchronize();
-  snprintf(name, sizeof(name), "conv_tc%s kind%d amode%d N%d %dx%d K%d N%d nt%d epi%d mode%d", g_f16 ? " f16" : "", kind, a_mode, N, H, W, gk, gn, nt, epi, p.epi_mode);
+  snprintf(name, sizeof(name), "conv_tc%s kind%d amode%d N%d %dx%d K%d N%d nt%d epi%d mode%d%s%s", g_f16 ? " f16" : "", kind, a_mode, N, H, W, gk, gn, nt,
+           epi, p.epi_mode, g_tile_rev ? " rev" : "", g_chunks == 1 ? " list" : (g_chunks == 2 ? " gap-list" : ""));
   if (rc == DASR_E_SMEM && e == cudaSuccess) {
     printf("[SKIP] %s (does not fit shared memory in this A mode)\n", name);
     return;
@@ -521,6 +537,36 @@
             printf("tma_%s row=%4d B rows/box=%3d pitch=%4d B : %8.1f cycles/box  %6.2f cycles/row  %6.2f B/clk/SM rc=%d\n",
                    store ? "store" : "load ", re * 2, rows, pitch * 2, c, c / rows, re * 2.0 * rows / c, rc);
           }
+      struct Mix { int ld_c, halo, nld, st_c, nst, cpa_c; const char* name; };
+      const Mix mixes[] = {
+          {32, 1, 1, 0, 0, 0, "(a) halo{32,10,18} loads"},
+          {64, 1, 1, 0, 0, 0, "(a) halo{64,10,18} loads"},
+          {64, 0, 1, 0, 0, 0, "(a) block{64,8,16} loads"},
+          {32, 0, 1, 0, 0, 0, "(a) block{32,8,16} loads"},
+          {0, 0, 0, 64, 1, 0, "(a) block{64,8,16} stores"},
+          {0, 0, 0, 32, 1, 0, "(a) block{32,8,16} stores"},
+          {32, 1, 1, 64, 1, 0, "(a) halo32 load + block64 store"},
+          {32, 1, 1, 32, 1, 0, "(a) halo32 load + block32 store"},
+          {64, 0, 1, 64, 1, 0, "(a) block64 load + block64 store"},
+          {32, 1, 2, 64, 1, 0, "(a) 2 halo32 loads + block64 store"},
+          {0, 0, 0, 0, 0, 64, "(b) cp.async 16 KB blocks alone"},
+          {0, 0, 0, 0, 0, 32, "(b) cp.async 8 KB blocks alone"},
+          {32, 1, 1, 0, 0, 64, "(b) halo32 loads | cp.async 16 KB"},
+          {32, 1, 1, 0, 0, 32, "(b) halo32 loads | cp.async 8 KB"},
+          {32, 1, 1, 64, 1, 64, "(b) halo32 load + block64 store | cp.async 16 KB"},
+      };
+      for (const Mix& m : mixes) {
+        double ct = 0, cc = 0;
+        const int iters = 400;
+        int rc = dasr_probe_tma_mix(m.ld_c, m.halo, m.nld, m.st_c, m.nst, m.cpa_c, iters, &ct, &cc);
+        const int rows = (m.ld_c ? m.nld * (m.halo ? 180 : 128) : 0) + (m.st_c ? m.nst * 128 : 0);
+        const double bytes = (m.ld_c ? m.nld * m.ld_c * 2.0 * (m.halo ? 180 : 128) : 0) + (m.st_c ? m.nst * m.st_c * 2.0 * 128 : 0);
+        printf("tma_mix %-48s : TMA %3d rows/iter %7.1f cyc/iter %5.2f cyc/row %6.2f B/clk/SM", m.name, rows, ct,
+               rows ? ct / rows : 0.0, ct > 0 ? bytes / ct : 0.0);
+        if (m.cpa_c) printf(" | cp.async 128 rows x %3d B %7.1f cyc/iter %5.2f cyc/row %6.2f B/clk/SM", m.cpa_c * 2, cc, cc / 128,
+                            m.cpa_c * 2.0 * 128 / cc);
+        printf(" rc=%d\n", rc);
+      }
       return 0;
     }
     if (!strcmp(argv[i], "mmarate")) {
@@ -659,6 +705,21 @@
         test_tc(1, 20, 13, 96, 192, 96, 0, 0, 4);
         test_tc(1, 16, 16, 512, 64, 32, 0, 0, 4);
         test_tc(1, 16, 16, 128, 64, 64, 1, 0, 4);
+        for (g_chunks = 1; g_chunks <= 2; g_chunks++) {
+          test_tc(1, 16, 8, 64, 192, 192, 0, 0, 4);
+          test_tc(1, 19, 11, 64, 96, 96, 0, 0, 4);
+          test_tc(1, 20, 13, 128, 64, 64, 0, 0, 5);
+          test_tc(3, 48, 40, 64, 64, 64, 0, 0, 5);
+          test_tc(2, 40, 24, 64, 32, 32, 0, 0, 5);
+          test_tc(2, 24, 16, 160, 32, 160, 1, 0, 7);
+          test_tc(1, 20, 13, 128, 32, 128, 1, 0, 7);
+          g_tile_rev = 1;
+          test_tc(1, 19, 11, 64, 192, 192, 0, 0, 4);
+          test_tc(1, 20, 13, 96, 64, 64, 0, 0, 5);
+          test_tc(1, 20, 13, 128, 96, 96, 0, 0, 5);
+          g_tile_rev = 0;
+        }
+        g_chunks = 0;
         g_f16 = 1;
         test_tc(2, 32, 16, 64, 192, 192, 0, 0, 4);
         test_tc(1, 20, 13, 96, 64, 64, 0, 0, 5);
```

Measured after the change: 276.0, median of 6. 0.737x the previous value.
